# LPD-EPFL-ML/X-MAP

Measured on AMD Instinct MI355X. Metric: item_sim_pairs_per_s, higher is better.
Workload: dtype f64

## Files before the change

include/xmap_hip.h:

```cpp
#ifndef XMAP_HIP_H
#define XMAP_HIP_H
#include <stdint.h>

#ifdef __cplusplus
extern "C" {
#endif

#define XMAP_OK 0
#define XMAP_ERR_HIP -1
#define XMAP_ERR_ARG -2
#define XMAP_ERR_OVERFLOW -3
#define XMAP_ERR_CAPACITY -4

#define XMAP_COSINE 0
#define XMAP_ADJUST_COSINE 1
#define XMAP_COSINE_EXACT 2

#define XMAP_TOPC 10

typedef struct xmap_ratings {
    int64_t n_users;
    int32_t n_items;
    int64_t nnz;
    const int64_t *user_ptr;
    const int32_t *user_item;
    const float *user_rating;
    const int64_t *user_time;
    const int64_t *item_ptr;
    const int32_t *item_user;
    const float *item_rating;
    const int32_t *prefix_cls;
    const int32_t *suffix_cls;
    const uint32_t *contains_mask;
    const uint8_t *flags;
} xmap_ratings;

const char *xmap_last_error(void);
int xmap_version(void);

int xmap_trim(void);
int xmap_debug_arena(void *stream, int64_t *live, int64_t *reserved);
int xmap_debug_arena_call(void *stream, int64_t bytes, int fail);

int xmap_exclusive_scan_i64(void *stream, const int64_t *in, int64_t *out, int64_t n, int64_t *h_total);
int xmap_exclusive_scan_i32_to_i64(void *stream, const int32_t *in, int64_t *out, int64_t n, int64_t *h_total);


int xmap_build_csc(void *stream, int64_t n_users, int32_t n_items, int64_t nnz, const int64_t *user_ptr,
                   const int32_t *user_item, const float *user_rating, int32_t *cnt ,
                   int64_t *item_ptr , int32_t *item_user , float *item_rating );

int xmap_user_stats(void *stream, const xmap_ratings *R, double *u_avg, double *u_norm2);

int xmap_item_stats(void *stream, const xmap_ratings *R, const double *u_avg, double *info ,
                    double *norms ,
                    int32_t *ua_item , int32_t *ia_user ,
                    int32_t item_lo, int32_t item_hi );

#ifdef XMAP_CROSSCHECK
int xmap_sim_plan(void *stream, const xmap_ratings *R, int32_t slot_target, int32_t *Q, int64_t *W, int64_t *unit_ptr,
                  int64_t *h_n_units, int64_t *h_contrib);
int xmap_sim_units(void *stream, int32_t n_items, const int32_t *Q, const int64_t *unit_ptr,
                   int32_t *unit_item , int32_t *unit_q );

int xmap_sim_count(void *stream, const xmap_ratings *R, int method, int cap, const double *u_avg,
                   const double *info, const int32_t *ua_item, const int32_t *ia_user, const int32_t *Q,
                   const int32_t *unit_item, const int32_t *unit_q, int64_t unit_lo, int64_t unit_hi,
                   int32_t *unit_cnt , int64_t *d_counters , int64_t *h_counters );
int xmap_sim_fill(void *stream, const xmap_ratings *R, int method, int cap, const double *u_avg,
                  const double *info, const int32_t *ua_item, const int32_t *ia_user, const int32_t *Q,
                  const int32_t *unit_item, const int32_t *unit_q, int64_t unit_lo, int64_t unit_hi,
                  const int64_t *unit_off , int32_t *col, double *sim, int32_t *mutu, int32_t *nij);

int xmap_sim_row_ptr(void *stream, int32_t n_items, const int64_t *unit_ptr, const int64_t *unit_off ,
                     int64_t *row_ptr );
#endif

int xmap_sim2_layout(void *stream, const xmap_ratings *R, const double *info, int32_t ch_min, int32_t *hist ,
                     int64_t *pre , int32_t *ctl , int32_t *hid , int32_t *hlist ,
                     uint64_t *ub_key , void *ub ,
                     void *rc ,
                     uint64_t *Wp ,
                     int32_t dups , int32_t *h_ctl );
int xmap_sim2_plan(void *stream, const xmap_ratings *R, int32_t slot_target, const void *rc, const int64_t *pre,
                   const int32_t *hid, const int32_t *ctl, int32_t *Q, int32_t *C, uint8_t *small ,
                   uint64_t *Wp , int32_t *Qcat , int64_t *uq_ptr ,
                   int64_t *uc_ptr , int32_t dups, int64_t *h_counts );
int xmap_sim2_units(void *stream, int32_t n_items, const int64_t *item_ptr, const int32_t *Qcat, const int64_t *uq_ptr,
                    int32_t *uq_item, int32_t *uq_q , const int32_t *C, const int64_t *uc_ptr, int32_t *uc_item,
                    int32_t *uc_c);
int xmap_sim2_pairs(void *stream, const xmap_ratings *R, int method, int cap, const double *u_avg, const double *norms,
                    const void *rc, const void *ub, const int32_t *Q,
                    const uint8_t *small, const int32_t *uq_item, const int32_t *uq_q, const int64_t *cls_ptr ,
                    int64_t unit_lo, int64_t unit_hi, const int32_t *hid,
                    const int32_t *hlist, const int32_t *ctl, const int32_t *C, const int64_t *uc_ptr,
                    const int32_t *uc_item, const int32_t *uc_c, int32_t n_heavy_units, int32_t n_heavy, int phases,
                    double *hp_hi, double *hp_lo, int32_t *hp_cnt, int32_t *hp_mut, int64_t coo_cap, int32_t *coo_i,
                    int32_t *coo_j, double *coo_sim, int32_t *coo_mutu, int32_t *coo_nij,
                    double *coo_ls , int32_t *rowcnt,
                    int32_t *rowcnt_h , int64_t *d_shards ,
                    int64_t *d_counters ,
                    int32_t *mircnt );
int xmap_sim2_scatter(void *stream, int32_t n_items, int64_t n_coo, const int32_t *coo_i, const int32_t *coo_j,
                      const double *coo_sim, const int32_t *coo_mutu, const int32_t *coo_nij, const double *coo_ls ,
                      const int64_t *row_ptr, int32_t *fill , const int32_t *hid, const int32_t *hlist,
                      int32_t *col, double *sim, int32_t *mutu, int32_t *nij, double *ls );
int xmap_sim3_layout(void *stream, const xmap_ratings *R, int64_t *item_ptr ,
                     const double *rating64 , int32_t ch_min, int32_t phases, int32_t stats_lo, int32_t stats_hi,
                     int32_t *cnt ,
                     double *u_avg , double *u_norm , int32_t *hist ,
                     int64_t *pre , int32_t *ctl , int32_t *hid , int32_t *hlist ,
                     uint64_t *ub_key , void *ub , void *srec ,
                     void *bufA , void *bufB , void *rc ,
                     uint64_t *Wp , double *info , double *norms , int32_t *h_ctl );
int xmap_sim3_plan(void *stream, const xmap_ratings *R, int32_t slot_target, const int64_t *pre, const int32_t *hid,
                   const int32_t *ctl, int32_t *Q, int32_t *C, uint8_t *small, uint64_t *Wp, int32_t *Qcat ,
                   int64_t *uq_ptr , int64_t *uc_ptr , int32_t dups, int32_t *uq_item, int32_t *uq_q ,
                   int32_t *uc_item, int32_t *uc_c, int64_t cap_light, int64_t cap_heavy, int64_t *h_out );
int xmap_sim3_mircount(void *stream, int32_t n_items, int64_t coo_cap, const int32_t *coo_i, const int32_t *coo_j,
                       const int64_t *d_shards , int64_t n_pairs, int32_t skip_self, void *scratch, int32_t *mir );
int xmap_sim3_mirror(void *stream, int32_t n_items, int64_t coo_cap, const int32_t *coo_i, const int32_t *coo_j,
                     const double *coo_sim, const int32_t *coo_mutu, const int32_t *coo_nij,
                     const int64_t *d_shards ,
                     int64_t n_pairs, const int32_t *own , const int32_t *mir , int32_t *tot ,
                     int64_t *row_ptr , int64_t *mptr , int32_t *fill ,
                     void *bufA , void *bufB , int32_t *col,
                     double *sim, int32_t *mutu, int32_t *nij, const double *coo_aux , double *aux ,
                     int32_t row_lo, int32_t row_hi );

int xmap_sim2_pack_pairs(void *stream, int64_t n_coo, const int32_t *coo_i, const int32_t *coo_j, const double *coo_sim,
                         const int32_t *coo_mutu, const int32_t *coo_nij, int64_t *rec , int64_t *h_count);
int xmap_sim2_unpack_pairs(void *stream, int64_t n, const int64_t *rec , int32_t *coo_i, int32_t *coo_j, double *coo_sim,
                           int32_t *coo_mutu, int32_t *coo_nij);
int xmap_item_partials(void *stream, const xmap_ratings *R, const double *u_avg, double *partial );
int xmap_item_merge(void *stream, int32_t n_items, int32_t n_parts, const double *parts , double *info ,
                    double *norms );
int xmap_sim2_pack_partials(void *stream, int64_t n_coo, const int32_t *coo_i, const int32_t *coo_j, const double *coo_hi,
                            const double *coo_lo, const int32_t *coo_mutu, const int32_t *coo_nij, int64_t *rec ,
                            int64_t *h_count);
int xmap_sim2_sort_partials(void *stream, int64_t n, const int64_t *rec , int64_t *rec_sorted , int32_t n_items,
                            int32_t n_owners );
int xmap_sim2_merge_partials(void *stream, int method, int cap, int32_t n_items, int64_t n, const int64_t *rec_sorted,
                             const double *norms , int32_t *coo_i, int32_t *coo_j, double *coo_sim, int32_t *coo_mutu,
                             int32_t *coo_nij, int32_t *rowcnt , int64_t *h_counts );



typedef struct xmap_sim {
    int32_t n_items;
    const int64_t *row_ptr;
    const int32_t *col;
    const double *sim;
    const int32_t *mutu;
    const int32_t *nij;
    const double *info;
    const double *frac;
} xmap_sim;

int xmap_bridge_flags(void *stream, const xmap_sim *S, const int32_t *prefix_cls, uint8_t *bb);

int xmap_knn_classify(void *stream, const xmap_sim *S, int top_k, const uint8_t *bb, const int32_t *suffix_cls,
                      const uint32_t *contains_mask, uint8_t *cls, int32_t *kcnt ,
                      int32_t *kcol , double *kval ,
                      int32_t row_lo, int32_t row_hi );

int xmap_knn_thresholds(void *stream, int32_t n_items, int top_k, const int32_t *kcnt, const int32_t *kcol, const double *kval,
                        void *thr );
int xmap_reverse_count(void *stream, const xmap_sim *S, int mode, int top_k, const uint8_t *bb, const uint8_t *cls,
                       const int32_t *kcnt, const int32_t *kcol, const double *kval, const int32_t *suffix_cls,
                       const uint32_t *contains_mask, const uint8_t *flags, const int64_t *attach_ptr,
                       const void *thr ,
                       int32_t *long_rows ,
                       uint8_t *eflag ,
                       int32_t *rcnt , int32_t row_lo, int32_t row_hi );
int xmap_reverse_count_att_rnn(void *stream, const xmap_sim *S, int top_k, const uint8_t *bb, const uint8_t *cls,
                               const int32_t *kcnt, const int32_t *kcol, const double *kval, const int32_t *suffix_cls,
                               const uint32_t *contains_mask, const uint8_t *flags, const void *thr, int32_t *long_rows,
                               uint8_t *eflag, int32_t *rcnt_att , int32_t *rcnt_rnn , int32_t row_lo, int32_t row_hi);
int xmap_reverse_fill(void *stream, const xmap_sim *S, int mode, int top_k, const uint8_t *bb, const uint8_t *cls,
                      const int32_t *kcnt, const int32_t *kcol, const double *kval, const int32_t *suffix_cls,
                      const uint32_t *contains_mask, const uint8_t *flags, const int64_t *attach_ptr,
                      const void *thr ,
                      int32_t *long_rows ,
                      uint8_t *eflag , const int64_t *rptr ,
                      int32_t *ridx, double *rval , uint8_t *rflag, int32_t row_lo, int32_t row_hi);

int xmap_path_weights(void *stream, int32_t n_items, int top_k, const uint8_t *cls, const int32_t *kcnt,
                      const int32_t *kcol, const uint8_t *flags, const int64_t *att_ptr, const int32_t *att_idx,
                      const int64_t *src_ptr, const int32_t *src_idx, const uint8_t *src_flag, const int64_t *rnn_ptr,
                      const int32_t *rnn_idx, int64_t *tmp , int64_t *paths );

int xmap_extend_paths(void *stream, int32_t n_items, int top_k, const uint8_t *cls, const int32_t *kcnt,
                      const int32_t *kcol, const double *kval, const uint8_t *flags, const int64_t *att_ptr,
                      const int32_t *att_idx, const double *att_val, const int64_t *src_ptr, const int32_t *src_idx,
                      const double *src_val, const uint8_t *src_flag, const int64_t *rnn_ptr, const int32_t *rnn_idx,
                      const double *rnn_val, int32_t n_units, const int32_t *unit_start, const int32_t *unit_c,
                      const int32_t *unit_G, const int32_t *unit_row, int32_t *unit_nt, int32_t n_heavy,
                      const int32_t *heavy_unit0, int32_t n_slots, double *acc, int32_t *touched, double *hacc,
                      int32_t *htouched, int32_t *n_cand, int32_t *top_end, double *top_val, int64_t xs_cap,
                      int64_t *xs_off, int32_t *xs_end, double *xs_val, int64_t *d_counters ,
                      int64_t *h_counters );
// ... 158 lines not shown
```

x-map_amd/csrc/api.hip:

```cpp
#include <math.h>
#include <stdlib.h>
#include <vector>

#include "common.h"

namespace xmap {

struct Pool {
    std::vector<void *> ptrs;
    void release() {
        for (void *p : ptrs) (void)hipFree(p);
        ptrs.clear();
    }
};

}

using namespace xmap;

struct xmap_ctx {
    int device = 0;
    hipStream_t st = nullptr;
    Pool p_ratings, p_sim, p_ext, p_gen, p_rows;
    xmap_ratings R;
// ... 177 lines not shown
        const double r = fabs((double)rating[k]);
        if (!(r <= 1e300)) return false;
        if (r > M) M = r;
        while (e <= 26 && ldexp(r, e) != floor(ldexp(r, e))) e++;
        if (e > 26) return false;
    }
    if (M == 0.0) return true;
    const double Mi = ldexp(M, e);
    if (Mi > 134217728.0) return false;
    const uint64_t m2 = (uint64_t)Mi * (uint64_t)Mi;
    return (uint64_t)U <= (1ull << 53) / m2;
}

int xmap_ctx_upload_ratings(xmap_ctx *c, int64_t n_users, int32_t n_items, const int64_t *user_ptr, const int32_t *item,
                            const float *rating, const int64_t *time, const int32_t *prefix_cls, const int32_t *suffix_cls,
                            const uint32_t *contains_mask, const uint8_t *flags) {
    XM_ARG(c && user_ptr && prefix_cls && suffix_cls && contains_mask && flags && n_users >= 0 && n_items >= 0);
    XM_HIP(hipSetDevice(c->device));
    drop_tail(c);
    c->p_gen.release(); c->p_ext.release(); c->p_sim.release(); c->p_ratings.release();
    c->have_sim = c->have_ext = c->have_gen = false;
    const int64_t nnz = user_ptr[n_users];
    XM_ARG(nnz >= 0 && nnz < 2147483647ll && (nnz == 0 || (item && rating && time)));
    for (int64_t e = 0; e < nnz; e++) XM_ARG(item[e] >= 0 && item[e] < n_items);
    xmap_ratings &R = c->R;
    memset(&R, 0, sizeof(R));
    R.n_users = n_users; R.n_items = n_items; R.nnz = nnz;
    c->half_contrib = 0;
    for (int64_t u = 0; u < n_users; u++) { const int64_t d = user_ptr[u + 1] - user_ptr[u]; c->half_contrib += d * (d - 1) / 2; }
    int64_t *d_ptr, *d_time, *d_iptr;
    int32_t *d_item, *d_iuser, *d_pre, *d_suf;
    float *d_rating, *d_irating;
    uint32_t *d_mask;
    uint8_t *d_flags;
    XM_TRY(h2d(c->p_ratings, &d_ptr, user_ptr, (size_t)n_users + 1, c->st));
    XM_TRY(h2d(c->p_ratings, &d_item, item, (size_t)nnz, c->st));
    XM_TRY(h2d(c->p_ratings, &d_rating, rating, (size_t)nnz, c->st));
    XM_TRY(h2d(c->p_ratings, &d_time, time, (size_t)nnz, c->st));
    XM_TRY(h2d(c->p_ratings, &d_pre, prefix_cls, (size_t)n_items, c->st));
    XM_TRY(h2d(c->p_ratings, &d_suf, suffix_cls, (size_t)n_items, c->st));
    XM_TRY(h2d(c->p_ratings, &d_mask, contains_mask, (size_t)n_items, c->st));
    XM_TRY(h2d(c->p_ratings, &d_flags, flags, (size_t)n_items, c->st));
    XM_ALLOCZ(c->p_ratings, d_iptr, n_items + 1);
    XM_ALLOCZ(c->p_ratings, d_iuser, nnz);
    XM_ALLOCZ(c->p_ratings, d_irating, nnz);
    R.user_ptr = d_ptr; R.user_item = d_item; R.user_rating = d_rating; R.user_time = d_time;
    R.item_ptr = d_iptr; R.item_user = d_iuser; R.item_rating = d_irating;
    R.prefix_cls = d_pre; R.suffix_cls = d_suf; R.contains_mask = d_mask; R.flags = d_flags;
    c->plain_exact = plain_sums_exact(n_users, nnz, rating);
    XM_HIP(hipStreamSynchronize(c->st));
    c->have_ratings = true;
    return XMAP_OK;
}

int xmap_ctx_item_sim(xmap_ctx *c, int method, int cap, int64_t *n_kept, int64_t *n_evaluated) {
    XM_ARG(c && c->have_ratings && (method == XMAP_COSINE || method == XMAP_ADJUST_COSINE) && cap > 0);
    XM_HIP(hipSetDevice(c->device));
    drop_tail(c);
    c->p_gen.release(); c->p_ext.release(); c->p_sim.release();
    c->have_sim = c->have_ext = c->have_gen = false;
    xmap_ratings &R = c->R;
    const int I = R.n_items;
    const int64_t U = R.n_users, nnz = R.nnz;
    const int pair_method = (method == XMAP_COSINE && !c->plain_exact) ? XMAP_COSINE_EXACT : method;
    Pool tmp;
    struct Guard { Pool &p; ~Guard() { p.release(); } } guard{tmp};
#define T_ALLOC(ptr, n) XM_TRY(dalloc(tmp, &(ptr), (size_t)(n), c->st))
#define T_ALLOCZ(ptr, n) XM_TRY(dalloc(tmp, &(ptr), (size_t)(n), c->st, true))
    int32_t *cnt;
    T_ALLOC(cnt, I);
    double *norms;
    XM_ALLOC(c->p_sim, c->u_avg, U);
    XM_ALLOC(c->p_sim, c->u_norm, U);
    XM_ALLOCZ(c->p_sim, c->info, (size_t)I * 4);
    T_ALLOCZ(norms, (size_t)2 * I);
    int32_t *hist, *ctl, *hid, *hlist;
    int64_t *pre;
    uint64_t *ub_key, *ub, *rcrec, *Wp, *srec, *buf_a, *buf_b;
    const size_t n1 = (size_t)(nnz ? nnz : 1);
    T_ALLOC(hist, U + 2); T_ALLOC(pre, U + 3); T_ALLOC(ctl, 4); T_ALLOC(hid, I); T_ALLOCZ(hlist, 1024);
    T_ALLOC(ub_key, n1); T_ALLOC(ub, n1); T_ALLOC(rcrec, 2 * n1); T_ALLOC(Wp, I);
    T_ALLOC(srec, 2 * n1); T_ALLOC(buf_a, 2 * n1); T_ALLOC(buf_b, 2 * n1);
    const int ch_min = 2048;
    XM_TRY(xmap_sim3_layout(c->st, &R, (int64_t *)R.item_ptr, nullptr, ch_min, 1 | 2 | 4, 0, I, cnt, c->u_avg, c->u_norm, hist, pre, ctl,
                            hid, hlist, ub_key, ub, srec, buf_a, buf_b, rcrec, Wp, c->info, norms, nullptr));
    const int64_t half_contrib = c->half_contrib;
    int32_t *Q, *Cc, *Qcat, *uq_item = nullptr, *uq_q = nullptr, *uc_item = nullptr, *uc_c = nullptr;
    uint8_t *small;
    int64_t *uq_ptr, *uc_ptr;
    T_ALLOCZ(Q, I); T_ALLOCZ(Cc, I); T_ALLOCZ(small, I); T_ALLOC(Qcat, (size_t)5 * (I ? I : 1)); T_ALLOCZ(uq_ptr, (size_t)5 * I + 1);
    T_ALLOCZ(uc_ptr, I + 1);
    int slot_target = 768;
    double coo_slack = 1.0;
    int64_t hc[10];
    int64_t n_light = 0, n_hu = 0;
    int n_heavy = 0;
    auto plan = [&](int target) -> int {
        const int64_t cap_light = half_contrib / target + I + 1, cap_heavy = nnz / ch_min + 1025;
        T_ALLOC(uq_item, cap_light); T_ALLOC(uq_q, 4 * cap_light); T_ALLOC(uc_item, cap_heavy); T_ALLOC(uc_c, cap_heavy);
        XM_TRY(xmap_sim3_plan(c->st, &R, target, pre, hid, ctl, Q, Cc, small, Wp, Qcat, uq_ptr, uc_ptr, 0, uq_item, uq_q, uc_item, uc_c,
                              cap_light, cap_heavy, hc));
        n_light = hc[0]; n_hu = hc[1]; n_heavy = (int)hc[9];
        return XMAP_OK;
    };
    XM_TRY(plan(slot_target));
    int32_t *coo_i = nullptr, *coo_j = nullptr, *coo_mutu = nullptr, *coo_nij = nullptr, *own = nullptr, *mir = nullptr;
    double *coo_sim = nullptr;
    int64_t *d_shards = nullptr;
    int64_t cap_coo = 0, n = 0, n_unordered = 0;
    for (;;) {
        cap_coo = ((int64_t)((double)(half_contrib > 0 ? half_contrib : 1) * coo_slack) / 4096 + 1100) * 4096;
        double *hp_hi, *hp_lo;
        int32_t *hp_cnt, *hp_mut, *rowcnt_h;
        int64_t *d_cnt;
        T_ALLOC(coo_i, cap_coo); T_ALLOC(coo_j, cap_coo); T_ALLOC(coo_sim, cap_coo); T_ALLOC(coo_mutu, cap_coo); T_ALLOC(coo_nij, cap_coo);
        T_ALLOC(own, I); T_ALLOC(mir, I);
        const size_t hp = (size_t)(n_hu ? n_hu : 1) * 1024;
        T_ALLOC(hp_hi, hp); T_ALLOC(hp_lo, hp); T_ALLOC(hp_cnt, hp); T_ALLOC(hp_mut, hp);
        T_ALLOCZ(d_cnt, 6); T_ALLOC(d_shards, 2 * 4096); T_ALLOC(rowcnt_h, 64 * 1024);
        XM_TRY(xmap_sim2_pairs(c->st, &R, pair_method, cap, c->u_avg, norms, rcrec, ub, Q, small, uq_item, uq_q, hc + 2, 0, n_light, hid, hlist,
                               ctl, Cc, uc_ptr, uc_item, uc_c, (int32_t)n_hu, n_heavy, 8 | 1 | 2 | 4 | 16 | 64 | 128, hp_hi, hp_lo, hp_cnt,
                               hp_mut, cap_coo, coo_i, coo_j, coo_sim, coo_mutu, coo_nij, nullptr, own, rowcnt_h, d_shards, d_cnt, mir));
        int64_t h_cnt[6];
        XM_TRY(d2h(h_cnt, d_cnt, 6, c->st));
        XM_HIP(hipStreamSynchronize(c->st));
        if (h_cnt[2]) {
            if (slot_target <= 32) { set_error("pair-table overflow"); return XMAP_ERR_OVERFLOW; }
            slot_target /= 2;
            XM_TRY(plan(slot_target));
            continue;
        }
        if (h_cnt[3]) {
            if (coo_slack > 64) { set_error("half-COO overflow"); return XMAP_ERR_CAPACITY; }
            coo_slack *= 2;
            continue;
        }
        n = h_cnt[4]; n_unordered = h_cnt[5];
        break;
    }
    int64_t *row_ptr, *mptr;
    XM_ALLOCZ(c->p_sim, row_ptr, I + 1);
    T_ALLOCZ(mptr, I + 1);
    const int64_t kept = 2 * n;
    int32_t *col, *mutu, *nij, *fill, *tot;
    double *sim;
    uint64_t *mir_a, *mir_b;
    XM_ALLOC(c->p_sim, col, kept); XM_ALLOC(c->p_sim, sim, kept); XM_ALLOC(c->p_sim, mutu, kept); XM_ALLOC(c->p_sim, nij, kept);
    T_ALLOC(fill, I); T_ALLOC(tot, I); T_ALLOC(mir_a, (size_t)3 * (n ? n : 1)); T_ALLOC(mir_b, (size_t)3 * (n ? n : 1));
    XM_TRY(xmap_sim3_mircount(c->st, I, cap_coo, coo_i, coo_j, d_shards, n, 0, mir_a, mir));
    XM_TRY(xmap_sim3_mirror(c->st, I, cap_coo, coo_i, coo_j, coo_sim, coo_mutu, coo_nij, d_shards, n, own, mir, tot, row_ptr, mptr, fill,
                            mir_a, mir_b, col, sim, mutu, nij, nullptr, nullptr, 0, I));
    XM_HIP(hipStreamSynchronize(c->st));
    c->S.n_items = I; c->S.row_ptr = row_ptr; c->S.col = col; c->S.sim = sim; c->S.mutu = mutu; c->S.nij = nij; c->S.info = c->info;
    c->S.frac = nullptr;
    c->n_kept = kept; c->n_eval = 2 * n_unordered; c->n_contrib = 2 * half_contrib;
    c->have_sim = true;
    if (n_kept) *n_kept = kept;
    if (n_evaluated) *n_evaluated = c->n_eval;
    return XMAP_OK;
#undef T_ALLOC
#undef T_ALLOCZ
}

int xmap_ctx_sim_download(xmap_ctx *c, int64_t *row_ptr, int32_t *col, double *sim, int32_t *mutu, int32_t *nij, double *info,
                          double *user_avg) {
    XM_ARG(c && c->have_sim);
    XM_HIP(hipSetDevice(c->device));
    const int I = c->R.n_items;
    if (row_ptr) XM_TRY(d2h(row_ptr, c->S.row_ptr, (size_t)I + 1, c->st));
    if (col) XM_TRY(d2h(col, c->S.col, (size_t)c->n_kept, c->st));
    if (sim) XM_TRY(d2h(sim, c->S.sim, (size_t)c->n_kept, c->st));
    if (mutu) XM_TRY(d2h(mutu, c->S.mutu, (size_t)c->n_kept, c->st));
    if (nij) XM_TRY(d2h(nij, c->S.nij, (size_t)c->n_kept, c->st));
    if (info) XM_TRY(d2h(info, (const double *)c->info, (size_t)I * 4, c->st));
    if (user_avg) XM_TRY(d2h(user_avg, (const double *)c->u_avg, (size_t)c->R.n_users, c->st));
    XM_HIP(hipStreamSynchronize(c->st));
    return XMAP_OK;
}

int xmap_ctx_extend(xmap_ctx *c, int top_k, int64_t *n_out, int64_t *n_paths) {
    XM_ARG(c && c->have_sim && top_k >= 1);
    XM_HIP(hipSetDevice(c->device));
    drop_tail(c);
    c->p_gen.release(); c->p_ext.release();
    c->have_ext = c->have_gen = false;
    const int I = c->R.n_items, k = top_k;
    c->top_k = k;
    xmap_ext_tables &T = c->T;
    memset(&T, 0, sizeof(T));
    T.n_items = I; T.top_k = k; T.flags = c->R.flags;
    XM_ALLOCZ(c->p_ext, c->n_cand, I);
    XM_ALLOC(c->p_ext, c->top_end, (size_t)I * XMAP_TOPC);
    XM_ALLOCZ(c->p_ext, c->top_val, (size_t)I * XMAP_TOPC);
    c->n_out = c->n_paths = 0;
    if (I == 0) { c->have_ext = true; if (n_out) *n_out = 0; if (n_paths) *n_paths = 0; return XMAP_OK; }
    uint8_t *bb, *cls;
    int32_t *kcnt, *kcol;
    double *kval;
    XM_ALLOCZ(c->p_ext, bb, I); XM_ALLOC(c->p_ext, cls, I); XM_ALLOC(c->p_ext, kcnt, (size_t)I * 2);
    XM_ALLOC(c->p_ext, kcol, (size_t)I * 2 * k); XM_ALLOC(c->p_ext, kval, (size_t)I * 2 * k * 3);
    XM_TRY(xmap_bridge_flags(c->st, &c->S, c->R.prefix_cls, bb));
    XM_TRY(xmap_knn_classify(c->st, &c->S, k, bb, c->R.suffix_cls, c->R.contains_mask, cls, kcnt, kcol, kval, 0, I));
    T.cls = cls; T.kcnt = kcnt; T.kcol = kcol; T.kval = kval;
    XM_TRY(xmap_edge_ranges(c->st, &c->S, &c->fast_div));
    double *thr;
    int32_t *long_rows;
    XM_ALLOC(c->p_ext, thr, (size_t)I * 4);
    XM_ALLOC(c->p_ext, long_rows, I + 1);
    uint8_t *eflag;
    XM_ALLOC(c->p_ext, eflag, (size_t)(c->n_kept > 0 ? c->n_kept : 1));
    XM_TRY(xmap_knn_thresholds(c->st, I, k, kcnt, kcol, kval, thr));
    const uint8_t *dummy;
    int32_t *cnt_att, *cnt_rnn;
    XM_ALLOCZ(c->p_ext, cnt_att, I);
    XM_ALLOCZ(c->p_ext, cnt_rnn, I);
    XM_TRY(xmap_reverse_count_att_rnn(c->st, &c->S, k, bb, cls, kcnt, kcol, kval, c->R.suffix_cls, c->R.contains_mask, c->R.flags,
                                      thr, long_rows, eflag, cnt_att, cnt_rnn, 0, I));
    XM_TRY(reverse_list(c, 0, bb, nullptr, thr, long_rows, eflag, cnt_att, &T.att_ptr, &T.att_idx, &T.att_val, &dummy));
    XM_TRY(reverse_list(c, 2, bb, nullptr, thr, long_rows, eflag, cnt_rnn, &T.rnn_ptr, &T.rnn_idx, &T.rnn_val, &dummy));
    XM_TRY(reverse_list(c, 1, bb, T.att_ptr, thr, long_rows, eflag, nullptr, &T.src_ptr, &T.src_idx, &T.src_val, &T.src_flag));
    int64_t *wtmp, *P;
    XM_ALLOCZ(c->p_ext, wtmp, (size_t)4 * I); XM_ALLOCZ(c->p_ext, P, I);
    XM_TRY(xmap_path_weights(c->st, I, k, cls, kcnt, kcol, c->R.flags, T.att_ptr, T.att_idx, T.src_ptr, T.src_idx, T.src_flag, T.rnn_ptr,
                             T.rnn_idx, wtmp, P));
    int32_t *nb_list, *nb_id;
    int64_t n_nb = 0;
    XM_ALLOC(c->p_ext, nb_list, I); XM_ALLOC(c->p_ext, nb_id, I);
    XM_TRY(xmap_nb_index(c->st, I, cls, nb_list, nb_id, &n_nb));
    T.n_nb = (int32_t)n_nb; T.nb_list = nb_list; T.nb_id = nb_id;
    if (n_nb > 0) {
        int32_t *ng;
        int64_t *nrec, *dir_ptr, *rec_ptr, n_tiles = 0, n_records = 0;
// ... 107 lines not shown
    const int64_t U = c->R.n_users;
    int32_t *d_top, *d_choice, *d_map, *d_picks = nullptr;
    XM_ALLOCZ(c->p_gen, d_top, I); XM_ALLOCZ(c->p_gen, d_choice, I); XM_ALLOCZ(c->p_gen, d_map, I);
    if (picks) XM_TRY(h2d(c->p_gen, &d_picks, picks, (size_t)I, c->st));
    XM_TRY(xmap_select_map(c->st, I, private_flag ? 1 : 0, c->n_cand, c->top_end, d_picks, d_top, d_choice, d_map));
    if (choice) XM_TRY(d2h(choice, (const int32_t *)d_choice, (size_t)I, c->st));
    int32_t *cnt_t, *cnt_m;
    int64_t *off_t, *off_m, nt = 0, nm = 0;
    XM_ALLOCZ(c->p_gen, cnt_t, U); XM_ALLOCZ(c->p_gen, cnt_m, U); XM_ALLOCZ(c->p_gen, off_t, U + 1); XM_ALLOCZ(c->p_gen, off_m, U + 1);
    XM_TRY(xmap_alterego_count(c->st, &c->R, d_map, cnt_t, cnt_m, nullptr));
    XM_TRY(xmap_exclusive_scan_i32_to_i64(c->st, cnt_t, off_t, U, &nt));
    XM_TRY(xmap_exclusive_scan_i32_to_i64(c->st, cnt_m, off_m, U, &nm));
    const int64_t n = nt + nm;
    XM_ALLOC(c->p_gen, c->g_user, n); XM_ALLOC(c->p_gen, c->g_item, n); XM_ALLOC(c->p_gen, c->g_rating, n); XM_ALLOC(c->p_gen, c->g_time, n);
    XM_TRY(xmap_alterego_fill(c->st, &c->R, d_map, off_t, off_m, nt, c->g_user, c->g_item, c->g_rating, c->g_time));
    XM_HIP(hipStreamSynchronize(c->st));
    c->n_rows = n; c->n_target_rows = nt;
    c->g_off_t = off_t; c->g_off_m = off_m;
    c->have_gen = true;
    if (n_rows) *n_rows = n;
    if (n_target_rows) *n_target_rows = nt;
    return XMAP_OK;
}

int xmap_ctx_gen_download(xmap_ctx *c, int32_t *user, int32_t *item, double *rating, int64_t *time) {
    XM_ARG(c && c->have_gen);
    XM_HIP(hipSetDevice(c->device));
    const size_t n = (size_t)c->n_rows;
    if (user) XM_TRY(d2h(user, (const int32_t *)c->g_user, n, c->st));
    if (item) XM_TRY(d2h(item, (const int32_t *)c->g_item, n, c->st));
    if (rating) XM_TRY(d2h(rating, (const double *)c->g_rating, n, c->st));
    if (time) XM_TRY(d2h(time, (const int64_t *)c->g_time, n, c->st));
    XM_HIP(hipStreamSynchronize(c->st));
    return XMAP_OK;
}


int xmap_ctx_rec_sim(xmap_ctx *c, int cap, int64_t *n_pairs) {
    XM_ARG(c && c->have_gen && cap > 0);
    XM_HIP(hipSetDevice(c->device));
    drop_tail(c);
    const int I = c->R.n_items;
    const int64_t U = c->R.n_users, nnz = c->n_rows;
    XM_ARG(nnz < 2147483647ll);
    const size_t n1 = (size_t)(nnz ? nnz : 1), i1 = (size_t)(I ? I : 1);
    XM_ALLOCZ(c->p_rec, c->pf_ptr, U + 1);
    XM_ALLOC(c->p_rec, c->pf_item, n1); XM_ALLOC(c->p_rec, c->pf_rating, n1); XM_ALLOC(c->p_rec, c->pf_time, n1);
    XM_TRY(xmap_rec_profiles(c->st, U, nnz, c->n_target_rows, c->g_off_t, c->g_off_m, c->g_user, c->g_item, c->g_rating, c->g_time,
                             c->pf_ptr, c->pf_item, c->pf_rating, c->pf_time));
    XM_ALLOCZ(c->p_rec, c->rs_row_ptr, I + 1);
    XM_ALLOCZ(c->p_rec, c->rs_avg, i1); XM_ALLOCZ(c->p_rec, c->rs_norm, i1);
    c->rec_pairs = 0;
    if (I == 0 || nnz == 0) {
        XM_HIP(hipStreamSynchronize(c->st));
        c->have_rec = true;
        if (n_pairs) *n_pairs = 0;
        return XMAP_OK;
    }
    std::vector<int64_t> h_ptr((size_t)U + 1);
    XM_TRY(d2h(h_ptr.data(), (const int64_t *)c->pf_ptr, (size_t)U + 1, c->st));
    XM_HIP(hipStreamSynchronize(c->st));
    int64_t half_contrib = 0;
    for (int64_t u = 0; u < U; u++) { const int64_t d = h_ptr[u + 1] - h_ptr[u]; half_contrib += d * (d - 1) / 2; }
    Pool tmp;
    struct Guard { Pool &p; ~Guard() { p.release(); } } guard{tmp};
#define T_ALLOC(ptr, n) XM_TRY(dalloc(tmp, &(ptr), (size_t)(n), c->st))
#define T_ALLOCZ(ptr, n) XM_TRY(dalloc(tmp, &(ptr), (size_t)(n), c->st, true))
    xmap_ratings P = c->R;
    float *f_dummy, *f_irating;
    int64_t *item_ptr;
    int32_t *i_user;
    T_ALLOCZ(f_dummy, n1); T_ALLOCZ(f_irating, n1); T_ALLOCZ(item_ptr, I + 1); T_ALLOCZ(i_user, n1);
    P.nnz = nnz; P.user_ptr = c->pf_ptr; P.user_item = c->pf_item; P.user_rating = f_dummy; P.user_time = c->pf_time;
    P.item_ptr = item_ptr; P.item_user = i_user; P.item_rating = f_irating;
    int32_t *cnt, *hist, *ctl, *hid, *hlist;
    int64_t *pre;
    uint64_t *ub_key, *ub, *rcrec, *Wp, *srec, *buf_a, *buf_b;
    double *u_avg, *info, *norms;
    T_ALLOC(cnt, i1); T_ALLOCZ(u_avg, U ? U : 1); T_ALLOCZ(info, i1 * 4); T_ALLOCZ(norms, 2 * i1);
    T_ALLOC(hist, U + 2); T_ALLOC(pre, U + 3); T_ALLOC(ctl, 4); T_ALLOC(hid, i1); T_ALLOCZ(hlist, 1024);
    T_ALLOC(ub_key, n1); T_ALLOC(ub, 2 * n1); T_ALLOC(rcrec, 2 * n1); T_ALLOC(Wp, i1);
    T_ALLOC(srec, 3 * n1); T_ALLOC(buf_a, 3 * n1); T_ALLOC(buf_b, 3 * n1);
    const int ch_min = (int)((U + 2 > 64) ? U + 2 : 64);
    XM_TRY(xmap_sim3_layout(c->st, &P, item_ptr, c->pf_rating, ch_min, 1 | 2 | 4, 0, I, cnt, u_avg, nullptr, hist, pre, ctl, hid, hlist,
                            ub_key, ub, srec, buf_a, buf_b, rcrec, Wp, info, norms, nullptr));
    int32_t *Q, *Cc, *Qcat, *uq_item = nullptr, *uq_q = nullptr, *uc_item = nullptr, *uc_c = nullptr;
    uint8_t *small;
    int64_t *uq_ptr, *uc_ptr;
    T_ALLOCZ(Q, i1); T_ALLOCZ(Cc, i1); T_ALLOCZ(small, i1); T_ALLOC(Qcat, 5 * i1); T_ALLOCZ(uq_ptr, (size_t)5 * I + 1);
    T_ALLOCZ(uc_ptr, I + 1);
    int slot_target = 768;
    double coo_slack = 1.0;
    int64_t hc[10];
    int64_t n_light = 0;
    auto plan = [&](int target) -> int {
        const int64_t cap_light = half_contrib / target + I + 1, cap_heavy = nnz / ch_min + 1025;
        T_ALLOC(uq_item, cap_light); T_ALLOC(uq_q, 4 * cap_light); T_ALLOC(uc_item, cap_heavy); T_ALLOC(uc_c, cap_heavy);
        XM_TRY(xmap_sim3_plan(c->st, &P, target, pre, hid, ctl, Q, Cc, small, Wp, Qcat, uq_ptr, uc_ptr, 1, uq_item, uq_q, uc_item, uc_c,
                              cap_light, cap_heavy, hc));
        n_light = hc[0];
        return XMAP_OK;
    };
    XM_TRY(plan(slot_target));
    int32_t *coo_i = nullptr, *coo_j = nullptr, *coo_mutu = nullptr, *coo_nij = nullptr, *own = nullptr, *mir = nullptr;
    double *coo_sim = nullptr, *coo_ls = nullptr;
    int64_t *d_shards = nullptr;
    int64_t cap_coo = 0, n = 0;
    for (;;) {
        cap_coo = ((int64_t)((double)(half_contrib > 0 ? half_contrib : 1) * coo_slack) / 4096 + 1100) * 4096;
        double *hp_hi, *hp_lo;
        int32_t *hp_cnt, *hp_mut, *rowcnt_h;
        int64_t *d_cnt;
        T_ALLOC(coo_i, cap_coo); T_ALLOC(coo_j, cap_coo); T_ALLOC(coo_sim, cap_coo); T_ALLOC(coo_mutu, cap_coo); T_ALLOC(coo_nij, cap_coo);
        T_ALLOC(coo_ls, cap_coo); T_ALLOC(own, i1); T_ALLOC(mir, i1);
        T_ALLOC(hp_hi, 1024); T_ALLOC(hp_lo, 1024); T_ALLOC(hp_cnt, 1024); T_ALLOC(hp_mut, 1024);
        T_ALLOCZ(d_cnt, 6); T_ALLOC(d_shards, 2 * 4096); T_ALLOC(rowcnt_h, 64 * 1024);
        XM_TRY(xmap_sim2_pairs(c->st, &P, XMAP_ADJUST_COSINE, cap, u_avg, norms, rcrec, ub, Q, small, uq_item, uq_q, hc + 2, 0, n_light, hid,
                               hlist, ctl, Cc, uc_ptr, uc_item, uc_c, 0, 0, 8 | 2 | 16 | 64 | 128, hp_hi, hp_lo, hp_cnt, hp_mut, cap_coo,
                               coo_i, coo_j, coo_sim, coo_mutu, coo_nij, coo_ls, own, rowcnt_h, d_shards, d_cnt, mir));
        int64_t h_cnt[6];
        XM_TRY(d2h(h_cnt, d_cnt, 6, c->st));
        XM_HIP(hipStreamSynchronize(c->st));
        if (h_cnt[2]) {
            if (slot_target <= 32) { set_error("pair-table overflow"); return XMAP_ERR_OVERFLOW; }
            slot_target /= 2;
            XM_TRY(plan(slot_target));
            continue;
        }
        if (h_cnt[3]) {
            if (coo_slack > 64) { set_error("half-COO overflow"); return XMAP_ERR_CAPACITY; }
            coo_slack *= 2;
            continue;
        }
        n = h_cnt[4];
        break;
    }
    int64_t *mptr;
    T_ALLOCZ(mptr, I + 1);
    const size_t kept_max = (size_t)(n ? 2 * n : 1), nn = (size_t)(n ? n : 1);
    int32_t *mutu, *fill, *tot;
    uint64_t *mir_a, *mir_b;
    XM_ALLOC(c->p_rec, c->rs_col, kept_max); XM_ALLOC(c->p_rec, c->rs_sim, kept_max); XM_ALLOC(c->p_rec, c->rs_nij, kept_max);
    XM_ALLOC(c->p_rec, c->rs_ls, kept_max);
    T_ALLOC(mutu, kept_max); T_ALLOC(fill, i1); T_ALLOC(tot, i1); T_ALLOC(mir_a, 4 * nn); T_ALLOC(mir_b, 4 * nn);
    XM_TRY(xmap_sim3_mircount(c->st, I, cap_coo, coo_i, coo_j, d_shards, n, 1, mir_a, mir));
    XM_TRY(xmap_sim3_mirror(c->st, I, cap_coo, coo_i, coo_j, coo_sim, coo_mutu, coo_nij, d_shards, n, own, mir, tot, c->rs_row_ptr, mptr, fill,
                            mir_a, mir_b, c->rs_col, c->rs_sim, mutu, c->rs_nij, coo_ls, c->rs_ls, 0, I));
    XM_HIP(hipMemcpy2DAsync(c->rs_avg, sizeof(double), info, 4 * sizeof(double), sizeof(double), (size_t)I, hipMemcpyDeviceToDevice, c->st));
    XM_HIP(hipMemcpyAsync(c->rs_norm, norms + I, sizeof(double) * (size_t)I, hipMemcpyDeviceToDevice, c->st));
    int64_t kept = 0;
    XM_TRY(d2h(&kept, (const int64_t *)(c->rs_row_ptr + I), 1, c->st));
    XM_HIP(hipStreamSynchronize(c->st));
    c->rec_pairs = kept;
    c->have_rec = true;
    if (n_pairs) *n_pairs = kept;
    return XMAP_OK;
#undef T_ALLOC
#undef T_ALLOCZ
}

int xmap_ctx_rec_profiles_download(xmap_ctx *c, int64_t *prof_ptr, int32_t *prof_item, double *prof_rating, int64_t *prof_time) {
    XM_ARG(c && c->have_rec);
    XM_HIP(hipSetDevice(c->device));
    const size_t n = (size_t)c->n_rows;
    if (prof_ptr) XM_TRY(d2h(prof_ptr, (const int64_t *)c->pf_ptr, (size_t)c->R.n_users + 1, c->st));
    if (prof_item) XM_TRY(d2h(prof_item, (const int32_t *)c->pf_item, n, c->st));
    if (prof_rating) XM_TRY(d2h(prof_rating, (const double *)c->pf_rating, n, c->st));
    if (prof_time) XM_TRY(d2h(prof_time, (const int64_t *)c->pf_time, n, c->st));
    XM_HIP(hipStreamSynchronize(c->st));
    return XMAP_OK;
}

int xmap_ctx_rec_download(xmap_ctx *c, int64_t *row_ptr, int32_t *col, double *sim, double *ls, int32_t *nij, double *item_avg,
                          double *item_norm) {
    XM_ARG(c && c->have_rec);
    XM_HIP(hipSetDevice(c->device));
    const size_t I = (size_t)c->R.n_items, n = (size_t)c->rec_pairs;
    if (row_ptr) XM_TRY(d2h(row_ptr, (const int64_t *)c->rs_row_ptr, I + 1, c->st));
    if (col) XM_TRY(d2h(col, (const int32_t *)c->rs_col, n, c->st));
    if (sim) XM_TRY(d2h(sim, (const double *)c->rs_sim, n, c->st));
    if (ls) XM_TRY(d2h(ls, (const double *)c->rs_ls, n, c->st));
    if (nij) XM_TRY(d2h(nij, (const int32_t *)c->rs_nij, n, c->st));
    if (item_avg) XM_TRY(d2h(item_avg, (const double *)c->rs_avg, I, c->st));
    if (item_norm) XM_TRY(d2h(item_norm, (const double *)c->rs_norm, I, c->st));
    XM_HIP(hipStreamSynchronize(c->st));
    return XMAP_OK;
}

static int alloc_neighbors(xmap_ctx *c, int keep) {
    c->p_nb.release();
    c->have_nb = false;
    const size_t m = (size_t)(c->R.n_items ? c->R.n_items : 1) * keep;
    XM_ALLOCZ(c->p_nb, c->nb_cnt, c->R.n_items ? c->R.n_items : 1);
    XM_ALLOCZ(c->p_nb, c->nb_col, m); XM_ALLOCZ(c->p_nb, c->nb_sim, m); XM_ALLOCZ(c->p_nb, c->nb_ls, m);
    c->keep = keep;
    return XMAP_OK;
}

int xmap_ctx_rec_select(xmap_ctx *c, int keep) {
    XM_ARG(c && c->have_rec && keep >= 1 && keep <= 64);
    XM_HIP(hipSetDevice(c->device));
    XM_TRY(alloc_neighbors(c, keep));
    if (c->rec_pairs > 0)
        XM_TRY(xmap_rec_select(c->st, c->R.n_items, c->rs_row_ptr, c->rs_col, c->rs_sim, c->rs_ls, keep, c->nb_cnt, c->nb_col, c->nb_sim,
                               c->nb_ls));
    XM_HIP(hipStreamSynchronize(c->st));
    c->have_nb = true;
    return XMAP_OK;
}

int xmap_ctx_rec_set_neighbors(xmap_ctx *c, int keep, const int32_t *cnt, const int32_t *col, const double *sim) {
    XM_ARG(c && c->have_rec && keep >= 1 && keep <= 64 && cnt && col && sim);
    XM_HIP(hipSetDevice(c->device));
    const int I = c->R.n_items;
    for (int i = 0; i < I; i++) {
        XM_ARG(cnt[i] <= keep);
        for (int t = 0; t < cnt[i]; t++) XM_ARG(col[(size_t)i * keep + t] >= 0 && col[(size_t)i * keep + t] < I);
    }
    XM_TRY(alloc_neighbors(c, keep));
    const size_t m = (size_t)I * keep;
    if (I) {
        XM_HIP(hipMemcpyAsync(c->nb_cnt, cnt, sizeof(int32_t) * (size_t)I, hipMemcpyHostToDevice, c->st));
        XM_HIP(hipMemcpyAsync(c->nb_col, col, sizeof(int32_t) * m, hipMemcpyHostToDevice, c->st));
        XM_HIP(hipMemcpyAsync(c->nb_sim, sim, sizeof(double) * m, hipMemcpyHostToDevice, c->st));
    }
    XM_HIP(hipStreamSynchronize(c->st));
    c->have_nb = true;
    return XMAP_OK;
// ... 49 lines not shown
```

x-map_amd/csrc/common.h:

```cpp
#pragma once
#if defined(__HIP_DEVICE_COMPILE__) && !defined(__gfx950__)
#error "libxmap_hip is written for gfx950 (MI355X): build with --offload-arch=gfx950"
#endif
#include <hip/hip_runtime.h>
#include <stdint.h>
#include <stdio.h>
#include <string.h>

#include "../../include/xmap_hip.h"

namespace xmap {

void set_error(const char *fmt, ...);

#define XM_HIP(call)                                                                         \
    do {                                                                                     \
        hipError_t e_ = (call);                                                              \
        if (e_ != hipSuccess) {                                                              \
            xmap::set_error("%s:%d %s -> %s", __FILE__, __LINE__, #call, hipGetErrorString(e_)); \
            return XMAP_ERR_HIP;                                                             \
        }                                                                                    \
    } while (0)

#define XM_LAUNCH_CHECK() XM_HIP(hipGetLastError())

#define XM_ARG(cond)                                                        \
    do {                                                                    \
        if (!(cond)) {                                                      \
            xmap::set_error("%s:%d bad argument: %s", __FILE__, __LINE__, #cond); \
            return XMAP_ERR_ARG;                                            \
        }                                                                   \
    } while (0)

hipError_t xm_malloc_async(void **p, size_t bytes, hipStream_t st);
hipError_t xm_free_async(void *p, hipStream_t st);
struct XmScope {
    int dev; hipStream_t st; size_t live0; bool ok;
    explicit XmScope(hipStream_t st);
    ~XmScope();
    XmScope(const XmScope &) = delete;
    XmScope &operator=(const XmScope &) = delete;
};
#define XM_SCOPE(stream) xmap::XmScope xm_scope_((hipStream_t)(stream))
int radix_sort_pairs(hipStream_t st, unsigned long long *keys, int *vals, unsigned long long *keys_tmp, int *vals_tmp, long long n,
                     int bits);

constexpr int WAVE = 64;

__device__ __forceinline__ int lane_id() { return threadIdx.x & 63; }

__device__ __forceinline__ int rl32(int v, int l) { return __builtin_amdgcn_readlane(v, l); }
__device__ __forceinline__ float rlf(float v, int l) { return __int_as_float(rl32(__float_as_int(v), l)); }
__device__ __forceinline__ long long rl64(long long v, int l) {
    int lo = rl32((int)(v & 0xffffffffll), l), hi = rl32((int)(v >> 32), l);
    return ((long long)hi << 32) | (unsigned int)lo;
}
__device__ __forceinline__ double rld(double v, int l) {
    return __longlong_as_double(rl64(__double_as_longlong(v), l));
}
__device__ __forceinline__ int uniform(int v) { return __builtin_amdgcn_readfirstlane(v); }

__device__ __forceinline__ unsigned long long lanemask_lt() {
    return (1ull << lane_id()) - 1ull;
}

__device__ __forceinline__ double wave_sum(double v) {
#pragma unroll
    for (int m = 32; m >= 1; m >>= 1) v += __shfl_xor(v, m, 64);
    return v;
}
__device__ __forceinline__ long long wave_sum_ll(long long v) {
#pragma unroll
    for (int m = 32; m >= 1; m >>= 1) v += __shfl_xor(v, m, 64);
    return v;
}

__device__ __forceinline__ void dd_add(double &hi, double &lo, double x) {
    double s = hi + x;
    double bb = s - hi;
    double e = (hi - (s - bb)) + (x - bb);
    e += lo;
    double h2 = s + e;
    lo = e - (h2 - s);
    hi = h2;
}

template <int G>
__device__ __forceinline__ void dd_reduce(double &hi, double &lo) {
#pragma unroll
    for (int m = G / 2; m >= 1; m >>= 1) {
        double oh = __shfl_down(hi, m, G), ol = __shfl_down(lo, m, G);
        dd_add(hi, lo, oh);
        dd_add(hi, lo, ol);
    }
}

__device__ __forceinline__ uint32_t mix32(uint32_t h) {
    h ^= h >> 16; h *= 0x85EBCA6Bu; h ^= h >> 13; h *= 0xC2B2AE35u; h ^= h >> 16;
    return h;
}

}
```

x-map_amd/csrc/stage_a2.hip:

```cpp
#include <type_traits>

#include "common.h"
#include "item_stats.h"
#include "tilesort.h"

namespace xmap {

constexpr int T_LOG_SLOTS = 10;
constexpr int T_SLOTS = 1 << T_LOG_SLOTS;
constexpr int HMAX = 1024;
constexpr uint32_t T_EMPTY = 0xFFFFFFFFu;
constexpr int SMALL_BOUND = 96;
constexpr int MID_BOUND = 384;

constexpr int N_CLASSES = 5;
constexpr int WIDE_MIN = 2048;
__host__ __device__ __forceinline__ int class_rank(int cls) {
    return cls == 4 ? 0 : (cls == 0 ? 1 : (cls == 2 ? 2 : (cls == 3 ? 3 : 4)));
}

__device__ __forceinline__ unsigned long long wkey(int n, int item) {
    return ((unsigned long long)(unsigned)n << 32) | (unsigned)item;
}

// ... 923 lines not shown
    }
    base = ((unsigned long long)(unsigned)rl32((int)(base >> 32), 0) << 32) | (unsigned)rl32((int)(base & 0xffffffffull), 0);
    if (!keep) return;
    const long long p = (long long)base + __popcll(km & lanemask_lt());
    coo_i[p] = i; coo_j[p] = j; coo_sim[p] = simv; coo_mutu[p] = mm; coo_nij[p] = nn;
    atomicAdd(&rowcnt[i], 1);
    atomicAdd(&rowcnt[j], 1);
}


constexpr int CNT_SLOTS = 4096;
constexpr int CNT_CHUNK = 8192;
__device__ __forceinline__ int cnt_slot(int it) { return (int)(mix32((uint32_t)it) & (CNT_SLOTS - 1)); }

__global__ __launch_bounds__(256) void k_count3(long long nnz, const int *uitem, int *cnt) {
    __shared__ int tag[CNT_SLOTS], loc[CNT_SLOTS];
    for (int t = threadIdx.x; t < CNT_SLOTS; t += 256) { tag[t] = -1; loc[t] = 0; }
    __syncthreads();
    const long long e0 = (long long)blockIdx.x * CNT_CHUNK;
    for (int q = threadIdx.x; q < CNT_CHUNK; q += 256) {
        const long long e = e0 + q;
        if (e >= nnz) break;
        const int it = uitem[e];
        const int sl = cnt_slot(it);
        const int old = atomicCAS(&tag[sl], -1, it);
        if (old == -1 || old == it) atomicAdd(&loc[sl], 1); else atomicAdd(&cnt[it], 1);
    }
    __syncthreads();
    for (int t = threadIdx.x; t < CNT_SLOTS; t += 256)
        if (loc[t]) atomicAdd(&cnt[tag[t]], loc[t]);
}

constexpr int CB_MAX = 1024;
constexpr int CB_CHUNK = 8192;
constexpr int CB_WIN = 8192;
constexpr int CB_SPB = 4;
constexpr int CB_T = 1024;

__global__ __launch_bounds__(CB_MAX) void k_cb_scan(const unsigned *bcnt, long long *bptr, unsigned *bcur) {
    __shared__ long long ws[CB_MAX / 64];
    const int t = threadIdx.x, lane = t & 63, w = t >> 6;
    const long long c = bcnt[t];
    long long inc = c;
#pragma unroll
    for (int d = 1; d < 64; d <<= 1) { const long long o = __shfl_up(inc, d, 64); if (lane >= d) inc += o; }
    if (lane == 63) ws[w] = inc;
    __syncthreads();
    long long base = 0;
    for (int x = 0; x < w; x++) base += ws[x];
    bptr[t] = base + inc - c;
    if (t == CB_MAX - 1) bptr[CB_MAX] = base + inc;
    bcur[t] = 0u;
}

__global__ __launch_bounds__(CB_T) void k_cb_count(long long nnz, const int *part, int sh, const long long *bptr, int n_items, int *cnt) {
    __shared__ unsigned win[CB_WIN];
    __shared__ int s_b;
    if (nnz < 0) nnz = bptr[CB_MAX];
    const long long p0 = (long long)blockIdx.x * (CB_CHUNK * CB_SPB);
    if (p0 >= nnz) return;
    if (threadIdx.x == 0) {
        int lo = 0, hi = CB_MAX;
        while (hi - lo > 1) { const int mid = (lo + hi) >> 1; if (bptr[mid] <= p0) lo = mid; else hi = mid; }
        s_b = lo;
    }
    for (int t = threadIdx.x; t < CB_WIN; t += CB_T) win[t] = 0u;
    __syncthreads();
    const int item0 = s_b << sh;
#pragma unroll 4
    for (int q = threadIdx.x; q < CB_CHUNK * CB_SPB; q += CB_T) {
        const long long p = p0 + q;
        if (p >= nnz) break;
        const int it = part[p];
        const unsigned d = (unsigned)(it - item0);
        if (d < (unsigned)CB_WIN) atomicAdd(&win[d], 1u); else atomicAdd(&cnt[it], 1);
    }
    __syncthreads();
    for (int t = threadIdx.x; t < CB_WIN; t += CB_T)
        if (win[t] && item0 + t < n_items) atomicAdd(&cnt[item0 + t], (int)win[t]);
}

template <bool SELF>
__global__ __launch_bounds__(CB_T) void k_cbs_hist(long long range_cap, int n_ranges, const unsigned long long *cur, const int *coo_i,
                                                   const int *coo_j, int sh, unsigned *bcnt) {
    __shared__ unsigned h[CB_MAX];
    for (int t = threadIdx.x; t < CB_MAX; t += CB_T) h[t] = 0u;
    __syncthreads();
    const long long cpr = (range_cap + CB_CHUNK - 1) / CB_CHUNK;
#pragma unroll
    for (int sg = 0; sg < CB_SPB; sg++) {
        const long long g = (long long)blockIdx.x * CB_SPB + sg;
        const long long c = g / n_ranges;
        const int r = (int)(g - c * n_ranges);
        if (c >= cpr) break;
        const long long n = (cur && (long long)cur[r] < range_cap) ? (long long)cur[r] : range_cap;
        const long long b = (long long)r * range_cap;
#pragma unroll
        for (int q = 0; q < CB_CHUNK / CB_T; q++) {
            const long long e = c * CB_CHUNK + q * CB_T + threadIdx.x;
            if (e < n) {
                const int j = coo_j[b + e];
                if (!SELF || j != coo_i[b + e]) atomicAdd(&h[j >> sh], 1u);
            }
        }
    }
    __syncthreads();
    for (int t = threadIdx.x; t < CB_MAX; t += CB_T)
        if (h[t]) atomicAdd(&bcnt[t], h[t]);
}

template <bool SELF>
__global__ __launch_bounds__(CB_T) void k_cbs_scatter(long long range_cap, int n_ranges, const unsigned long long *cur, const int *coo_i,
                                                      const int *coo_j, int sh, const long long *bptr, unsigned *bcur, int *out) {
    static_assert(CB_T == CB_MAX, "one thread per bucket in the scan");
    __shared__ unsigned h[CB_MAX], off[CB_MAX + 1], wsum[CB_T / 64];
    __shared__ long long base[CB_MAX];
    __shared__ int stage[CB_CHUNK * CB_SPB];
    const int tid = threadIdx.x;
    h[tid] = 0u;
    __syncthreads();
    constexpr int EPT = CB_CHUNK / CB_T;
    const long long cpr = (range_cap + CB_CHUNK - 1) / CB_CHUNK;
    int it[CB_SPB][EPT];
    unsigned rk[CB_SPB][EPT];
#pragma unroll
    for (int sg = 0; sg < CB_SPB; sg++) {
        const long long g = (long long)blockIdx.x * CB_SPB + sg;
        const long long c = g / n_ranges;
        const int r = (int)(g - c * n_ranges);
        const long long n = (c < cpr) ? ((cur && (long long)cur[r] < range_cap) ? (long long)cur[r] : range_cap) : 0;
        const long long b = (long long)r * range_cap;
#pragma unroll
        for (int q = 0; q < EPT; q++) {
            const long long e = c * CB_CHUNK + q * CB_T + tid;
            it[sg][q] = -1;
            if (e < n) {
                const int j = coo_j[b + e];
                if (!SELF || j != coo_i[b + e]) it[sg][q] = j;
            }
        }
    }
#pragma unroll
    for (int sg = 0; sg < CB_SPB; sg++)
#pragma unroll
        for (int q = 0; q < EPT; q++) rk[sg][q] = it[sg][q] >= 0 ? atomicAdd(&h[it[sg][q] >> sh], 1u) : 0u;
    __syncthreads();
    {
        const unsigned c = h[tid];
        const int lane = tid & 63, w = tid >> 6;
        unsigned inc = c;
#pragma unroll
        for (int d = 1; d < 64; d <<= 1) { const unsigned o = __shfl_up(inc, d, 64); if (lane >= d) inc += o; }
        if (lane == 63) wsum[w] = inc;
        __syncthreads();
        unsigned bs = 0;
        for (int x = 0; x < w; x++) bs += wsum[x];
        off[tid] = bs + inc - c;
        if (tid == CB_T - 1) off[CB_MAX] = bs + inc;
        if (c) base[tid] = bptr[tid] + (long long)atomicAdd(&bcur[tid], c);
    }
    __syncthreads();
#pragma unroll
    for (int sg = 0; sg < CB_SPB; sg++)
#pragma unroll
        for (int q = 0; q < EPT; q++)
            if (it[sg][q] >= 0) stage[off[it[sg][q] >> sh] + rk[sg][q]] = it[sg][q];
    __syncthreads();
    const int total = (int)off[CB_MAX];
    for (int x = tid; x < total; x += CB_T) {
        const int v = stage[x];
        const int bk = v >> sh;
        out[base[bk] + (x - (int)off[bk])] = v;
    }
}


template <bool WIDE>
__device__ __forceinline__ void sort_entry3(const int *uitem, const float *ur32, const double *ur64, const int *cnt,
                                            long long e, unsigned long long &key, int &px, long long &py) {
    const int it = uitem[e];
    key = wkey(cnt[it], it);
    px = it;
    py = WIDE ? __double_as_longlong(ur64[e]) : (long long)(unsigned)__float_as_int(ur32[e]);
}

template <bool WIDE>
__device__ __forceinline__ void bitonic_desc3(int width, int pos, unsigned long long &key, int &px, long long &py) {
#pragma unroll
    for (int k2 = 2; k2 <= 64; k2 <<= 1) {
        if (k2 <= width)
#pragma unroll
        for (int j = k2 >> 1; j > 0; j >>= 1) {
            const unsigned long long ok = __shfl_xor(key, j, 64);
            const int ox = __shfl_xor(px, j, 64);
            long long oy;
            if (WIDE) oy = __shfl_xor(py, j, 64); else oy = (long long)(unsigned)__shfl_xor((int)py, j, 64);
            const bool desc = (pos & k2) == 0;
            const bool lower = (pos & j) == 0;
            const bool take_other = (lower == desc) ? (ok > key) : (ok < key);
            if (take_other) { key = ok; px = ox; py = oy; }
        }
    }
}

template <bool WIDE>
__device__ __forceinline__ void emit_entry3(long long a, int d, int rank, long long u, int px, long long py, void *ub,
                                            unsigned long long *srec) {
    const long long e = a + rank;
    const unsigned pos_ge = (unsigned)(d >= 2 ? rank : 0) | ((unsigned)px & 0x80000000u);
    const unsigned long long w0 = (unsigned long long)((unsigned)px & 0x7fffffffu) | ((unsigned long long)pos_ge << 32);
    if (WIDE) {
        UbWide v; v.item_ge = px; v.pad = 0; v.rating = __longlong_as_double(py);
        ((UbWide *)ub)[e] = v;
        srec[e * 3 + 0] = w0; srec[e * 3 + 1] = (unsigned long long)py; srec[e * 3 + 2] = (unsigned long long)(unsigned)u;
    } else {
        ((int2 *)ub)[e] = make_int2(px, (int)py);
        ulonglong2 w; w.x = w0; w.y = (unsigned long long)(unsigned)py | ((unsigned long long)(unsigned)u << 32);
        *(ulonglong2 *)(srec + e * 2) = w;
    }
}

// ... 471 lines not shown
    G.K = K; G.M = M; G.ch = ch;
    G.ts_log = 11;
    for (;;) {
        const long long TS = 1ll << G.ts_log;
        long long kw = M / (4 * (long long)(K > 0 ? K : 1));
        const long long kw_min = TS / (ts::NK_MAX - 2) + 1;
        if (kw < kw_min) kw = kw_min;
        if (kw < 4) kw = 4;
        const long long tiles = ((M + (long long)K * kw) >> G.ts_log) + 1;
        if (tiles <= (long long)ts::NA_MAX * ts::NB || G.ts_log >= 30) {
            G.KW = (int)kw;
            G.NA = (int)((tiles + ts::NB - 1) / ts::NB);
            if (G.NA < 1) G.NA = 1;
            if (G.NA > ts::NA_MAX) G.NA = ts::NA_MAX;
            G.T = G.NA * ts::NB;
            return;
        }
        G.ts_log++;
    }
}

int ts_prepare(hipStream_t st, ts::Geo &G, const long long *ptr) {
    G.ptr = ptr;
    G.clist_cap = G.M / G.ch + G.NA + 1;
    G.slist_cap = G.M / ts::SL + (G.M >> G.ts_log) + 2;
    XM_HIP(xm_malloc_async((void **)&G.tk, sizeof(unsigned) * (size_t)(G.K > 0 ? G.K : 1), st));
    XM_HIP(xm_malloc_async((void **)&G.tile_key0, sizeof(int) * ((size_t)G.T + 1), st));
    XM_HIP(xm_malloc_async((void **)&G.tile_pos0, sizeof(long long) * ((size_t)G.T + 1), st));
    XM_HIP(xm_malloc_async((void **)&G.tile_large, sizeof(int) * (size_t)G.T, st));
    unsigned long long *z = nullptr;
    const size_t nz = (size_t)G.NA + 2 * (size_t)G.T + 1;
    XM_HIP(xm_malloc_async((void **)&z, sizeof(unsigned long long) * nz, st));
    G.curA = z; G.curB = z + G.NA; G.counters = (unsigned *)(z + G.NA + 2 * (size_t)G.T);
    XM_HIP(xm_malloc_async((void **)&G.clist, sizeof(int2) * (size_t)G.clist_cap, st));
    XM_HIP(xm_malloc_async((void **)&G.slist, sizeof(int2) * (size_t)G.slist_cap, st));
    XM_HIP(hipMemsetAsync(z, 0, sizeof(unsigned long long) * nz, st));
    XM_HIP(hipMemsetAsync(G.tile_large, 0xff, sizeof(int) * (size_t)G.T, st));
    ts::k_ts_plan<<<dim3((unsigned)((G.K + 255) / 256)), dim3(256), 0, st>>>(G);
    XM_LAUNCH_CHECK();
    ts::k_ts_chunks<<<dim3((unsigned)((G.NA + 255) / 256)), dim3(256), 0, st>>>(G);
    XM_LAUNCH_CHECK();
    return XMAP_OK;
}
}

namespace {
template <bool AUX, bool SHARE>
int mirror_levels(hipStream_t st, const ts::Geo &G, int64_t coo_cap, const int32_t *coo_i, const int32_t *coo_j, const double *coo_sim,
                  const int32_t *coo_mutu, const int32_t *coo_nij, const double *coo_aux, const longlong2 *chunks, const unsigned *n_chunks,
                  long long chunk_cap, int64_t n_pairs, const int32_t *own, const int64_t *row_ptr, int32_t *fill, void *bufA, void *bufB,
                  int32_t *col, double *sim, int32_t *mutu, int32_t *nij, double *aux, int row_lo, int row_hi) {
    constexpr int RW = AUX ? 4 : 3;
    CooLoaderT<AUX, SHARE> LA{coo_i, coo_j, coo_sim, coo_mutu, coo_nij, coo_aux, chunks, n_chunks, (const long long *)row_ptr, fill,
                              col, sim, mutu, nij, aux, row_lo, row_hi};
    ts::RecLoader<RW> LB{(const unsigned long long *)bufA};
    ts::k_ts_bin<RW, false, CooLoaderT<AUX, SHARE>><<<dim3((unsigned)chunk_cap), dim3(ts::BT), 0, st>>>(G, LA, coo_cap, (unsigned long long *)bufA);
    XM_LAUNCH_CHECK();
    ts::k_ts_bin<RW, true, ts::RecLoader<RW>><<<dim3((unsigned)G.clist_cap), dim3(ts::BT), 0, st>>>(G, LB, n_pairs, (unsigned long long *)bufB);
    XM_LAUNCH_CHECK();
    k_mir_tiles<AUX><<<dim3((unsigned)G.T), dim3(ts::CT), 0, st>>>(G, (const unsigned long long *)bufB, (const long long *)row_ptr, own, col,
                                                                   sim, mutu, nij, aux);
    XM_LAUNCH_CHECK();
    k_mir_large<AUX><<<dim3((unsigned)G.slist_cap), dim3(ts::LT), 0, st>>>(G, (const unsigned long long *)bufB, (const long long *)row_ptr, own,
                                                                            col, sim, mutu, nij, aux);
    XM_LAUNCH_CHECK();
    return XMAP_OK;
}
}

namespace {
int mirror_counts(hipStream_t st, int n_items, long long range_cap, int n_ranges, const unsigned long long *cur, const int *coo_i,
                  const int *coo_j, bool skip_self, int *part, int *counts) {
    if (n_items <= 0 || range_cap <= 0 || n_ranges <= 0) return XMAP_OK;
    int sh = 0;
    while (((long long)(n_items - 1) >> sh) >= CB_MAX) sh++;
    unsigned *bcnt = nullptr, *bcur = nullptr;
    long long *bptr = nullptr;
    XM_HIP(xm_malloc_async((void **)&bcnt, sizeof(unsigned) * CB_MAX, st));
    XM_HIP(xm_malloc_async((void **)&bcur, sizeof(unsigned) * CB_MAX, st));
    XM_HIP(xm_malloc_async((void **)&bptr, sizeof(long long) * (CB_MAX + 1), st));
    XM_HIP(hipMemsetAsync(bcnt, 0, sizeof(unsigned) * CB_MAX, st));
    const long long segs = (long long)n_ranges * ((range_cap + CB_CHUNK - 1) / CB_CHUNK);
    const dim3 g((unsigned)((segs + CB_SPB - 1) / CB_SPB));
    if (skip_self) k_cbs_hist<true><<<g, dim3(CB_T), 0, st>>>(range_cap, n_ranges, cur, coo_i, coo_j, sh, bcnt);
    else k_cbs_hist<false><<<g, dim3(CB_T), 0, st>>>(range_cap, n_ranges, cur, coo_i, coo_j, sh, bcnt);
    XM_LAUNCH_CHECK();
    k_cb_scan<<<dim3(1), dim3(CB_MAX), 0, st>>>(bcnt, bptr, bcur);
    XM_LAUNCH_CHECK();
    if (skip_self) k_cbs_scatter<true><<<g, dim3(CB_T), 0, st>>>(range_cap, n_ranges, cur, coo_i, coo_j, sh, bptr, bcur, part);
    else k_cbs_scatter<false><<<g, dim3(CB_T), 0, st>>>(range_cap, n_ranges, cur, coo_i, coo_j, sh, bptr, bcur, part);
    XM_LAUNCH_CHECK();
    const long long cap = range_cap * n_ranges;
    k_cb_count<<<dim3((unsigned)((cap + (long long)CB_CHUNK * CB_SPB - 1) / ((long long)CB_CHUNK * CB_SPB))), dim3(CB_T), 0, st>>>(
        -1, part, sh, bptr, n_items, counts);
    XM_LAUNCH_CHECK();
    return XMAP_OK;
}
}

extern "C" {

int xmap_sim2_layout(void *stream, const xmap_ratings *R, const double *info, int32_t ch_min, int32_t *hist ,
                     int64_t *pre , int32_t *ctl , int32_t *hid, int32_t *hlist ,
                     uint64_t *ub_key , void *ub , void *rc ,
                     uint64_t *Wp , int32_t dups, int32_t *h_ctl ) {
    XM_ARG(R && info && hist && pre && ctl && hid && hlist && ub_key && ub && rc && Wp && ch_min >= 64);
    XM_ARG(R->nnz < 0x7fffffffLL && R->n_users < 0x7ffffff0LL);
    hipStream_t st = (hipStream_t)stream;
    const int I = R->n_items;
    const int HB = (int)R->n_users + 2;
    XM_HIP(hipMemsetAsync(hist, 0, sizeof(int32_t) * (size_t)HB, st));
    XM_HIP(hipMemsetAsync(ctl, 0x7f, sizeof(int32_t), st));
    XM_HIP(hipMemsetAsync(ctl + 1, 0, 3 * sizeof(int32_t), st));
    if (I > 0) {
        k_hist<<<dim3((unsigned)((I + 256 * HIST_PER - 1) / (256 * HIST_PER))), dim3(256), 0, st>>>(
            I, (const long long *)R->item_ptr, HB, hist);
        XM_LAUNCH_CHECK();
    }
    int rcode = xmap_exclusive_scan_i32_to_i64(stream, hist, pre, HB, nullptr);
    if (rcode) return rcode;
    if (HB - 1 > ch_min) {
        k_threshold<<<dim3((unsigned)((HB + 255) / 256)), dim3(256), 0, st>>>(I, HB, (const long long *)pre, ch_min, ctl);
        XM_LAUNCH_CHECK();
    }
    if (I > 0) {
        k_mark_heavy<<<dim3((unsigned)((I + 255) / 256)), dim3(256), 0, st>>>(I, (const long long *)R->item_ptr, ctl, hid,
                                                                                hlist, ctl + 1);
        XM_LAUNCH_CHECK();
    }
    if (R->n_users > 0) {
        k_sort_profiles<<<dim3((unsigned)((R->n_users + 15) / 16)), dim3(256), 0, st>>>(
            R->n_users, (const long long *)R->user_ptr, R->user_item, R->user_rating, (const long long *)R->item_ptr, info,
            (unsigned long long *)ub_key, (int2 *)ub);
        XM_LAUNCH_CHECK();
    }
    XM_HIP(hipMemsetAsync(Wp, 0, sizeof(uint64_t) * (size_t)(I > 0 ? I : 1), st));
    if (R->nnz > 0) {
        if (dups) XM_HIP(hipMemsetAsync(ub_key, 0, sizeof(int32_t) * (size_t)R->nnz, st));
        k_rater_records<<<dim3((unsigned)((R->nnz + 255) / 256)), dim3(256), 0, st>>>(
            I, R->nnz, (const long long *)R->item_ptr, R->item_user, (const long long *)R->user_ptr, (const int2 *)ub,
            (RaterRec *)rc, dups ? (int *)ub_key : nullptr, (unsigned long long *)Wp);
        XM_LAUNCH_CHECK();
    }
    if (h_ctl) {
        XM_HIP(hipMemcpyAsync(h_ctl, ctl, 2 * sizeof(int32_t), hipMemcpyDeviceToHost, st));
        XM_HIP(hipStreamSynchronize(st));
        if (h_ctl[1] > HMAX) {
            set_error("heavy set larger than %d", HMAX);
            return XMAP_ERR_OVERFLOW;
        }
    }
    return XMAP_OK;
}

int xmap_sim2_plan(void *stream, const xmap_ratings *R, int32_t slot_target, const void *rc, const int64_t *pre,
                   const int32_t *hid, const int32_t *ctl, int32_t *Q, int32_t *C, uint8_t *small, uint64_t *Wp ,
                   int32_t *Qcat , int64_t *uq_ptr , int64_t *uc_ptr, int32_t dups,
                   int64_t *h_counts ) {
    XM_ARG(R && rc && Wp && pre && hid && ctl && Q && C && small && Qcat && uq_ptr && uc_ptr && h_counts);
    XM_ARG(slot_target > 0 && slot_target <= T_SLOTS);
    hipStream_t st = (hipStream_t)stream;
    const int I = R->n_items;
    XM_HIP(hipMemsetAsync(Qcat, 0, sizeof(int32_t) * (size_t)N_CLASSES * (size_t)(I > 0 ? I : 1), st));
    if (I > 0) {
        k_plan2<<<dim3((unsigned)((I + 255) / 256)), dim3(256), 0, st>>>(
            I, (const long long *)R->item_ptr, (const RaterRec *)rc, (const long long *)pre, (int)R->n_users + 2, hid, ctl,
            slot_target, dups, Q, C, small, (unsigned long long *)Wp, Qcat);
        XM_LAUNCH_CHECK();
    }
    int rcode = xmap_exclusive_scan_i32_to_i64(stream, Qcat, uq_ptr, (int64_t)N_CLASSES * I, &h_counts[0]);
    if (rcode) return rcode;
    rcode = xmap_exclusive_scan_i32_to_i64(stream, C, uc_ptr, I, &h_counts[1]);
    if (rcode) return rcode;
    if (I > 0)
        XM_HIP(hipMemcpy2DAsync(&h_counts[2], sizeof(int64_t), uq_ptr, sizeof(int64_t) * (size_t)I, sizeof(int64_t),
                                N_CLASSES, hipMemcpyDeviceToHost, st));
    else
        for (int c = 0; c < N_CLASSES; c++) h_counts[2 + c] = 0;
    XM_HIP(hipStreamSynchronize(st));
    h_counts[2 + N_CLASSES] = h_counts[0];
    return XMAP_OK;
}

int xmap_sim2_units(void *stream, int32_t n_items, const int64_t *item_ptr, const int32_t *Qcat, const int64_t *uq_ptr,
                    int32_t *uq_item, int32_t *uq_q, const int32_t *C, const int64_t *uc_ptr, int32_t *uc_item, int32_t *uc_c) {
    XM_ARG(item_ptr && Qcat && uq_ptr && uq_item && uq_q && C && uc_ptr && uc_item && uc_c);
    if (n_items == 0) return XMAP_OK;
    k_fill_units2<<<dim3((unsigned)(((long long)N_CLASSES * n_items + 255) / 256)), dim3(256), 0, (hipStream_t)stream>>>(
        n_items, (const long long *)item_ptr, Qcat, (const long long *)uq_ptr, uq_item, uq_q, C, (const long long *)uc_ptr, uc_item, uc_c, 0x7fffffffffffffffLL,
        0x7fffffffffffffffLL);
    XM_LAUNCH_CHECK();
    return XMAP_OK;
}

int xmap_sim3_plan(void *stream, const xmap_ratings *R, int32_t slot_target, const int64_t *pre, const int32_t *hid,
                   const int32_t *ctl, int32_t *Q, int32_t *C, uint8_t *small, uint64_t *Wp, int32_t *Qcat, int64_t *uq_ptr,
                   int64_t *uc_ptr, int32_t dups, int32_t *uq_item, int32_t *uq_q, int32_t *uc_item, int32_t *uc_c,
                   int64_t cap_light, int64_t cap_heavy, int64_t *h_out) {
    XM_SCOPE(stream);
    XM_ARG(R && Wp && pre && hid && ctl && Q && C && small && Qcat && uq_ptr && uc_ptr && h_out);
    XM_ARG(uq_item && uq_q && uc_item && uc_c && cap_light >= 0 && cap_heavy >= 0);
    XM_ARG(slot_target > 0 && slot_target <= T_SLOTS);
    hipStream_t st = (hipStream_t)stream;
    const int I = R->n_items;
    for (int c = 0; c < 10; c++) h_out[c] = 0;
    XM_HIP(hipMemsetAsync(Qcat, 0, sizeof(int32_t) * (size_t)N_CLASSES * (size_t)(I > 0 ? I : 1), st));
    if (I > 0) {
        k_plan2<<<dim3((unsigned)((I + 255) / 256)), dim3(256), 0, st>>>(
            I, (const long long *)R->item_ptr, nullptr, (const long long *)pre, (int)R->n_users + 2, hid, ctl, slot_target, dups, Q, C,
            small, (unsigned long long *)Wp, Qcat);
        XM_LAUNCH_CHECK();
    }
    int rcode = xmap_exclusive_scan_i32_to_i64(stream, Qcat, uq_ptr, (int64_t)N_CLASSES * I, nullptr);
    if (rcode) return rcode;
    rcode = xmap_exclusive_scan_i32_to_i64(stream, C, uc_ptr, I, nullptr);
    if (rcode) return rcode;
    if (I > 0) {
        k_fill_units2<<<dim3((unsigned)(((long long)N_CLASSES * I + 255) / 256)), dim3(256), 0, st>>>(
            I, (const long long *)R->item_ptr, Qcat, (const long long *)uq_ptr, uq_item, uq_q, C, (const long long *)uc_ptr, uc_item, uc_c,
            cap_light, cap_heavy);
        XM_LAUNCH_CHECK();
        XM_HIP(hipMemcpy2DAsync(&h_out[2], sizeof(int64_t), uq_ptr, sizeof(int64_t) * (size_t)I, sizeof(int64_t), N_CLASSES + 1,
                                hipMemcpyDeviceToHost, st));
        XM_HIP(hipMemcpyAsync(&h_out[1], uc_ptr + I, sizeof(int64_t), hipMemcpyDeviceToHost, st));
    }
    int32_t h_ctl[2] = {0, 0};
    XM_HIP(hipMemcpyAsync(h_ctl, ctl, 2 * sizeof(int32_t), hipMemcpyDeviceToHost, st));
    XM_HIP(hipStreamSynchronize(st));
    h_out[0] = h_out[2 + N_CLASSES];
    h_out[8] = h_ctl[0]; h_out[9] = h_ctl[1];
    if (h_ctl[1] > HMAX) {
        set_error("heavy set larger than %d", HMAX);
        return XMAP_ERR_OVERFLOW;
    }
    if (h_out[0] > cap_light || h_out[1] > cap_heavy) {
        set_error("unit arrays too small: %lld light / %lld heavy units, room for %lld / %lld", (long long)h_out[0], (long long)h_out[1],
                  (long long)cap_light, (long long)cap_heavy);
        return XMAP_ERR_CAPACITY;
    }
    return XMAP_OK;
}

int xmap_sim2_pairs(void *stream, const xmap_ratings *R, int method, int cap, const double *u_avg, const double *norms,
                    const void *rc, const void *ub, const int32_t *Q,
                    const uint8_t *small, const int32_t *uq_item, const int32_t *uq_q, const int64_t *cls_ptr ,
                    int64_t unit_lo, int64_t unit_hi, const int32_t *hid,
                    const int32_t *hlist, const int32_t *ctl, const int32_t *C, const int64_t *uc_ptr,
                    const int32_t *uc_item, const int32_t *uc_c, int32_t n_heavy_units, int32_t n_heavy, int phases,
                    double *hp_hi, double *hp_lo, int32_t *hp_cnt, int32_t *hp_mut, int64_t coo_cap, int32_t *coo_i,
                    int32_t *coo_j, double *coo_sim, int32_t *coo_mutu, int32_t *coo_nij, double *coo_ls ,
                    int32_t *rowcnt, int32_t *rowcnt_h , int64_t *d_shards ,
                    int64_t *d_counters , int32_t *mircnt ) {
    XM_SCOPE(stream);
    XM_ARG(R && u_avg && norms && rc && ub);
    XM_ARG(Q && small && uq_item && uq_q && cls_ptr && hid && hlist && ctl && C && uc_ptr && uc_item && uc_c);
    XM_ARG(coo_i && coo_j && coo_sim && coo_mutu && coo_nij && rowcnt && rowcnt_h && d_shards && d_counters);
    XM_ARG(coo_cap >= COO_SHARDS);
    XM_ARG(method == XMAP_COSINE || method == XMAP_ADJUST_COSINE || method == XMAP_COSINE_EXACT);
    XM_ARG(n_heavy_units == 0 || !(phases & 5) || (hp_hi && hp_lo && hp_cnt && hp_mut));
    hipStream_t st = (hipStream_t)stream;
    const bool exact_cos = method == XMAP_COSINE_EXACT;
    const double *nrm = norms + (method == XMAP_ADJUST_COSINE ? (size_t)R->n_items : 0);
    if (exact_cos) {
        double *zero_avg = nullptr;
        const size_t ub = sizeof(double) * (size_t)(R->n_users > 0 ? R->n_users : 1);
        XM_HIP(xm_malloc_async((void **)&zero_avg, ub, st));
        XM_HIP(hipMemsetAsync(zero_avg, 0, ub, st));
        u_avg = zero_avg;
        method = XMAP_ADJUST_COSINE;
    }
    const bool raw = (phases & 32) != 0;
    XM_ARG(!coo_ls || ((raw || method == XMAP_ADJUST_COSINE) && n_heavy_units == 0));
    XM_ARG(!raw || (coo_ls && n_heavy_units == 0 && n_heavy == 0));
    if (phases & 8) {
        XM_HIP(hipMemsetAsync(d_counters, 0, 4 * sizeof(int64_t), st));
        XM_HIP(hipMemsetAsync(d_shards, 0, 2 * COO_SHARDS * sizeof(int64_t), st));
        if (!(phases & 128)) XM_HIP(hipMemsetAsync(coo_i, 0xff, sizeof(int32_t) * (size_t)coo_cap, st));
        XM_HIP(hipMemsetAsync(rowcnt, 0, sizeof(int32_t) * (size_t)(R->n_items > 0 ? R->n_items : 1), st));
        if (mircnt) XM_HIP(hipMemsetAsync(mircnt, 0, sizeof(int32_t) * (size_t)(R->n_items > 0 ? R->n_items : 1), st));
    }
    TriArgs A;
    memset(&A, 0, sizeof(A));
    A.iptr = (const long long *)R->item_ptr; A.rc = (const RaterRec *)rc; A.ub = (const int2 *)ub;
    A.u_avg = u_avg; A.nrm = nrm; A.cap = cap;
    A.Q = Q; A.small = small; A.uq_item = uq_item; A.uq_q = uq_q; A.unit_lo = unit_lo; A.unit_hi = unit_hi;
    A.hid = hid; A.hlist = hlist; A.CH = ctl; A.uc_item = uc_item; A.uc_c = uc_c;
    A.uc_ptr = (const long long *)uc_ptr; A.C = C;
    A.hp_hi = hp_hi; A.hp_lo = hp_lo; A.hp_cnt = hp_cnt; A.hp_mut = hp_mut;
    A.shard_cap = coo_cap / COO_SHARDS; A.shard_cur = (unsigned long long *)d_shards;
    A.shard_occ = (unsigned long long *)d_shards + COO_SHARDS; A.coo_i = coo_i; A.coo_j = coo_j; A.coo_sim = coo_sim; A.coo_mutu = coo_mutu; A.coo_nij = coo_nij;
    A.coo_aux = coo_ls;
    A.raw = raw ? 1 : 0;
    A.heavy_mod = (phases >> 16) & 0xff; A.heavy_rem = (phases >> 8) & 0xff;
    if (A.heavy_mod < 1) A.heavy_mod = 1;
    A.rowcnt = rowcnt; A.mircnt = mircnt; A.rowcnt_h = rowcnt_h; A.counters = (unsigned long long *)d_counters;
    const bool heavy_aside = (phases & 7) == 7 && n_heavy_units > 0 && unit_hi > unit_lo;
    hipStream_t hs = st;
    SideStreams *side = nullptr;
    if (((phases & 2) && unit_hi > unit_lo) || heavy_aside) {
        side = side_streams();
        if (!side) return XMAP_ERR_HIP;
        XM_HIP(hipEventRecord(side->fork, st));
    }
    if (heavy_aside) {
        hs = side->s[N_CLASSES];
        XM_HIP(hipStreamWaitEvent(hs, side->fork, 0));
    }
    if ((phases & 1) && n_heavy_units > 0) {
        if (method == XMAP_COSINE) k_pair_heavy<XMAP_COSINE><<<dim3((unsigned)n_heavy_units), dim3(64 * HEAVY_WAVES), 0, hs>>>(A);
        else k_pair_heavy<XMAP_ADJUST_COSINE><<<dim3((unsigned)n_heavy_units), dim3(64 * HEAVY_WAVES), 0, hs>>>(A);
        XM_LAUNCH_CHECK();
    }
    if (heavy_aside && n_heavy > 0) {
        if (method == XMAP_COSINE) k_heavy_merge<XMAP_COSINE><<<dim3((unsigned)n_heavy), dim3(256), 0, hs>>>(A, n_heavy);
        else k_heavy_merge<XMAP_ADJUST_COSINE><<<dim3((unsigned)n_heavy), dim3(256), 0, hs>>>(A, n_heavy);
        XM_LAUNCH_CHECK();
    }
    if (heavy_aside) {
        XM_HIP(hipEventRecord(side->done[N_CLASSES], hs));
        XM_HIP(hipStreamWaitEvent(st, side->done[N_CLASSES], 0));
    }
    if ((phases & 2) && unit_hi > unit_lo) {
        for (int c = 0; c < N_CLASSES; c++) {
// ... 262 lines not shown
            XM_LAUNCH_CHECK();
        }
    }
    }
    if ((phases & 2) && stats_hi > stats_lo) {
        BigList B;
        B.chunk_cap = nnz / STAT_CHK + nnz / STAT_BIG + 2;
        B.item_cap = nnz / STAT_BIG + 2;
        XM_HIP(xm_malloc_async((void **)&B.counters, 2 * sizeof(unsigned), st));
        XM_HIP(xm_malloc_async((void **)&B.chunks, sizeof(int2) * (size_t)B.chunk_cap, st));
        XM_HIP(xm_malloc_async((void **)&B.items, sizeof(int4) * (size_t)B.item_cap, st));
        XM_HIP(xm_malloc_async((void **)&B.part, sizeof(double) * ITEM_PART * (size_t)B.chunk_cap, st));
        XM_HIP(hipMemsetAsync(B.counters, 0, 2 * sizeof(unsigned), st));
        const dim3 grid((unsigned)((stats_hi - stats_lo + 15) / 16)), gridC((unsigned)((B.chunk_cap + 3) / 4)), gridI((unsigned)((B.item_cap + 63) / 64));
        if (wide) {
            const RcWideSrc src{(const RaterRecWide *)rc};
            k_item_stats3<RcWideSrc><<<grid, dim3(256), 0, st>>>(I, stats_lo, stats_hi, (const long long *)item_ptr, src, info, norms, B);
            XM_LAUNCH_CHECK();
            k_item_chunks<RcWideSrc><<<gridC, dim3(256), 0, st>>>((const long long *)item_ptr, src, B);
            XM_LAUNCH_CHECK();
            k_item_big<<<gridI, dim3(64), 0, st>>>(I, B, info, norms);
            XM_LAUNCH_CHECK();
        } else {
            const RcSrc src{(RaterRec *)rc, u_avg};
            k_item_stats3<RcSrc><<<grid, dim3(256), 0, st>>>(I, stats_lo, stats_hi, (const long long *)item_ptr, src, info, norms, B);
            XM_LAUNCH_CHECK();
            k_item_chunks<RcSrc><<<gridC, dim3(256), 0, st>>>((const long long *)item_ptr, src, B);
            XM_LAUNCH_CHECK();
            k_item_big<<<gridI, dim3(64), 0, st>>>(I, B, info, norms);
            XM_LAUNCH_CHECK();
            k_item_big_flags<RcSrc><<<gridC, dim3(256), 0, st>>>((const long long *)item_ptr, src, B, info);
            XM_LAUNCH_CHECK();
        }
    }
    if (!wide && nnz > 0 && I > 0) {
        if (phases & 8) {
            k_rc_flags<<<dim3((unsigned)((nnz + 255) / 256)), dim3(256), 0, st>>>(nnz, (RaterRec *)rc, (const int2 *)ub, info);
            XM_LAUNCH_CHECK();
        }
        if (phases & 4) {
            k_ub_flags<<<dim3((unsigned)((nnz + 255) / 256)), dim3(256), 0, st>>>(nnz, (int2 *)ub, info);
            XM_LAUNCH_CHECK();
        }
    }
    if (h_ctl) {
        XM_HIP(hipMemcpyAsync(h_ctl, ctl, 2 * sizeof(int32_t), hipMemcpyDeviceToHost, st));
        XM_HIP(hipStreamSynchronize(st));
        if (h_ctl[1] > HMAX) {
            set_error("heavy set larger than %d", HMAX);
            return XMAP_ERR_OVERFLOW;
        }
    }
    return XMAP_OK;
}

int xmap_sim3_mircount(void *stream, int32_t n_items, int64_t coo_cap, const int32_t *coo_i, const int32_t *coo_j,
                       const int64_t *d_shards, int64_t n_pairs, int32_t skip_self, void *scratch, int32_t *mir) {
    XM_SCOPE(stream);
    XM_ARG(coo_i && coo_j && scratch && mir && n_items >= 0 && coo_cap >= 0 && n_pairs >= 0);
    XM_ARG(d_shards ? (coo_cap >= COO_SHARDS) : (n_pairs <= coo_cap));
    hipStream_t st = (hipStream_t)stream;
    if (n_items == 0) return XMAP_OK;
    XM_HIP(hipMemsetAsync(mir, 0, sizeof(int32_t) * (size_t)n_items, st));
    if (n_pairs == 0 || coo_cap == 0) return XMAP_OK;
    if (d_shards)
        return mirror_counts(st, n_items, coo_cap / COO_SHARDS, COO_SHARDS, (const unsigned long long *)d_shards, coo_i, coo_j,
                             skip_self != 0, (int *)scratch, mir);
    return mirror_counts(st, n_items, n_pairs, 1, nullptr, coo_i, coo_j, skip_self != 0, (int *)scratch, mir);
}

int xmap_sim3_mirror(void *stream, int32_t n_items, int64_t coo_cap, const int32_t *coo_i, const int32_t *coo_j,
                     const double *coo_sim, const int32_t *coo_mutu, const int32_t *coo_nij, const int64_t *d_shards, int64_t n_pairs,
                     const int32_t *own, const int32_t *mir, int32_t *tot, int64_t *row_ptr, int64_t *mptr, int32_t *fill,
                     void *bufA, void *bufB, int32_t *col, double *sim, int32_t *mutu, int32_t *nij, const double *coo_aux, double *aux,
                     int32_t row_lo, int32_t row_hi) {
    XM_SCOPE(stream);
    XM_ARG(row_lo >= 0 && row_lo <= row_hi && row_hi <= n_items);
    XM_ARG(coo_i && coo_j && coo_sim && coo_mutu && coo_nij && own && mir && tot && row_ptr && mptr && fill && bufA && bufB);
    XM_ARG(col && sim && mutu && nij && n_items >= 0 && coo_cap >= 0 && n_pairs >= 0 && n_pairs < 0x7fffffffLL);
    XM_ARG(d_shards ? (coo_cap >= COO_SHARDS) : (n_pairs <= coo_cap));
    XM_ARG((coo_aux != nullptr) == (aux != nullptr));
    hipStream_t st = (hipStream_t)stream;
    const int I = n_items;
    if (I > 0) {
        k_row_totals<<<dim3((unsigned)((I + 255) / 256)), dim3(256), 0, st>>>(I, own, mir, tot);
        XM_LAUNCH_CHECK();
    }
    int rcode = xmap_exclusive_scan_i32_to_i64(stream, tot, row_ptr, I, nullptr);
    if (rcode) return rcode;
    rcode = xmap_exclusive_scan_i32_to_i64(stream, mir, mptr, I, nullptr);
    if (rcode) return rcode;
    if (n_pairs == 0 || I == 0 || coo_cap == 0) return XMAP_OK;
    XM_HIP(hipMemsetAsync(fill, 0, sizeof(int32_t) * (size_t)I, st));
    ts::Geo G;
    ts_geometry(I, n_pairs, coo_aux ? ts::Chunk<4>::CH : ts::Chunk<3>::CH, G);
    rcode = ts_prepare(st, G, (const long long *)mptr);
    if (rcode) return rcode;
    static_assert(ts::Chunk<3>::CH <= ts::Chunk<4>::CH && ts::Chunk<4>::CH % ts::Chunk<3>::CH == 0, "chunk lists by the narrow record width");
    const int n_shards = d_shards ? COO_SHARDS : 1;
    const long long shard_cap = d_shards ? coo_cap / COO_SHARDS : coo_cap;
    const long long chunk_cap = n_pairs / ts::Chunk<3>::CH + n_shards + 1;
    longlong2 *chunks = nullptr;
    unsigned *n_chunks = nullptr;
    XM_HIP(xm_malloc_async((void **)&chunks, sizeof(longlong2) * (size_t)chunk_cap, st));
    XM_HIP(xm_malloc_async((void **)&n_chunks, sizeof(unsigned), st));
    XM_HIP(hipMemsetAsync(n_chunks, 0, sizeof(unsigned), st));
    k_coo_chunks<<<dim3((unsigned)((n_shards + 255) / 256)), dim3(256), 0, st>>>(n_shards, shard_cap, (const unsigned long long *)d_shards,
                                                                                 n_pairs, chunks, n_chunks, chunk_cap);
    XM_LAUNCH_CHECK();
    const bool share = row_lo > 0 || row_hi < I;
#define XM_MIRROR(AUX_, SHARE_, CA_, A_) mirror_levels<AUX_, SHARE_>(st, G, coo_cap, coo_i, coo_j, coo_sim, coo_mutu, coo_nij, CA_, chunks, n_chunks, \
        chunk_cap, n_pairs, own, row_ptr, fill, bufA, bufB, col, sim, mutu, nij, A_, row_lo, row_hi)
    if (coo_aux) return share ? XM_MIRROR(true, true, coo_aux, aux) : XM_MIRROR(true, false, coo_aux, aux);
    return share ? XM_MIRROR(false, true, nullptr, nullptr) : XM_MIRROR(false, false, nullptr, nullptr);
#undef XM_MIRROR
}
}
```

x-map_amd/csrc/util.hip:

```cpp
#include <stdarg.h>
#include <stdlib.h>
#include <vector>

#include "common.h"

namespace xmap {
static thread_local char g_err[512] = "";
void set_error(const char *fmt, ...) {
    va_list ap;
    va_start(ap, fmt);
    vsnprintf(g_err, sizeof(g_err), fmt, ap);
    va_end(ap);
}

namespace {
struct Chunk { char *base; size_t size, used; };
struct Arena { int dev; hipStream_t st; std::vector<Chunk> chunks; size_t live; };
thread_local std::vector<Arena> g_arenas;
constexpr size_t ARENA_KEEP = (size_t)256 << 20;
Arena *arena_find(int dev, hipStream_t st) {
    for (Arena &a : g_arenas) if (a.dev == dev && a.st == st) return &a;
    return nullptr;
}
Arena *arena_of(hipStream_t st) {
    int dev = 0;
    if (hipGetDevice(&dev) != hipSuccess) return nullptr;
    if (Arena *a = arena_find(dev, st)) return a;
    g_arenas.push_back(Arena{dev, st, {}, 0});
    return &g_arenas.back();
}
void arena_reset(Arena *a) {
    size_t total = 0;
    for (Chunk &c : a->chunks) { c.used = 0; total += c.size; }
    if (total <= ARENA_KEEP) return;
    if (hipStreamSynchronize(a->st) != hipSuccess) return;
    std::vector<Chunk> keep;
    size_t kept = 0;
    std::vector<Chunk> all = a->chunks;
    for (size_t i = 0; i < all.size(); i++)
        for (size_t j = i + 1; j < all.size(); j++)
            if (all[j].size < all[i].size) { Chunk t = all[i]; all[i] = all[j]; all[j] = t; }
    for (Chunk &c : all) {
        if (kept + c.size <= ARENA_KEEP) { keep.push_back(c); kept += c.size; }
        else (void)hipFree(c.base);
    }
    a->chunks.swap(keep);
}
}

XmScope::XmScope(hipStream_t s) : dev(0), st(s), live0(0), ok(false) {
    if (hipGetDevice(&dev) != hipSuccess) return;
    ok = true;
    if (Arena *a = arena_find(dev, st)) live0 = a->live;
}
XmScope::~XmScope() {
    if (!ok) return;
    Arena *a = arena_find(dev, st);
    if (!a || a->live <= live0) return;
    a->live = live0;
    if (a->live == 0) arena_reset(a);
}

hipError_t xm_malloc_async(void **p, size_t bytes, hipStream_t st) {
    Arena *a = arena_of(st);
    if (!a) return hipErrorInvalidDevice;
    bytes = (bytes + 255) & ~(size_t)255;
    if (bytes == 0) bytes = 256;
    for (Chunk &c : a->chunks)
        if (c.size - c.used >= bytes) { *p = c.base + c.used; c.used += bytes; a->live++; return hipSuccess; }
    Chunk c;
    c.size = bytes > ((size_t)32 << 20) ? bytes : ((size_t)32 << 20);
    c.used = bytes;
    hipError_t e = hipMalloc((void **)&c.base, c.size);
    if (e != hipSuccess) return e;
    a->chunks.push_back(c);
    *p = c.base;
    a->live++;
    return hipSuccess;
}
hipError_t xm_free_async(void *p, hipStream_t st) {
    (void)p;
    Arena *a = arena_of(st);
    if (!a || a->live == 0) return hipErrorInvalidValue;
    if (--a->live == 0) arena_reset(a);
    return hipSuccess;
}

constexpr int SCAN_THREADS = 256;
constexpr int SCAN_ITEMS = 8;
constexpr int SCAN_TILE = SCAN_THREADS * SCAN_ITEMS;

__device__ __forceinline__ long long block_exclusive_scan(long long v, long long *total, long long *smem) {
    int lane = threadIdx.x & 63, w = threadIdx.x >> 6;
    long long inc = v;
#pragma unroll
    for (int d = 1; d < 64; d <<= 1) {
        long long o = __shfl_up(inc, d, 64);
        if (lane >= d) inc += o;
    }
    if (lane == 63) smem[w] = inc;
    __syncthreads();
    long long base = 0, tot = 0;
    for (int k = 0; k < SCAN_THREADS / 64; k++) {
        long long s = smem[k];
        if (k < w) base += s;
        tot += s;
    }
    __syncthreads();
    *total = tot;
    return base + inc - v;
}

template <typename TIn>
__global__ __launch_bounds__(SCAN_THREADS) void k_tile_sums(const TIn *in, long long n, long long *tile_sum) {
    __shared__ long long smem[4];
    long long base = (long long)blockIdx.x * SCAN_TILE + (long long)threadIdx.x * SCAN_ITEMS;
    long long s = 0;
#pragma unroll
    for (int k = 0; k < SCAN_ITEMS; k++)
        if (base + k < n) s += (long long)in[base + k];
    long long tot;
    block_exclusive_scan(s, &tot, smem);
    if (threadIdx.x == 0) tile_sum[blockIdx.x] = tot;
}

__global__ __launch_bounds__(SCAN_THREADS) void k_scan_tile_sums(long long *tile_sum, long long n_tiles, long long *grand) {
    __shared__ long long smem[4];
    long long carry = 0;
    for (long long b = 0; b < n_tiles; b += SCAN_THREADS) {
        long long i = b + threadIdx.x;
        long long v = i < n_tiles ? tile_sum[i] : 0;
        long long tot;
        long long ex = block_exclusive_scan(v, &tot, smem);
        if (i < n_tiles) tile_sum[i] = carry + ex;
        carry += tot;
    }
    if (threadIdx.x == 0) *grand = carry;
}

template <typename TIn>
__global__ __launch_bounds__(SCAN_THREADS) void k_tile_scan(const TIn *in, long long n, const long long *tile_off,
                                                            long long *out) {
    __shared__ long long smem[4];
    long long base = (long long)blockIdx.x * SCAN_TILE + (long long)threadIdx.x * SCAN_ITEMS;
    long long v[SCAN_ITEMS];
    long long s = 0;
#pragma unroll
    for (int k = 0; k < SCAN_ITEMS; k++) {
        v[k] = (base + k < n) ? (long long)in[base + k] : 0;
        s += v[k];
    }
    long long tot;
    long long ex = block_exclusive_scan(s, &tot, smem) + tile_off[blockIdx.x];
#pragma unroll
    for (int k = 0; k < SCAN_ITEMS; k++) {
        if (base + k < n) out[base + k] = ex;
        ex += v[k];
    }
}

template <typename TIn>
static int exclusive_scan(hipStream_t st, const TIn *in, int64_t *out, int64_t n, int64_t *h_total) {
    XM_ARG(n >= 0);
    XM_SCOPE(st);
    int64_t n_tiles = (n + SCAN_TILE - 1) / SCAN_TILE;
    long long *tile = nullptr;
    XM_HIP(xm_malloc_async((void **)&tile, sizeof(long long) * (size_t)(n_tiles + 1), st));
    if (n_tiles > 0) {
        k_tile_sums<TIn><<<dim3((unsigned)n_tiles), dim3(SCAN_THREADS), 0, st>>>(in, n, tile);
        XM_LAUNCH_CHECK();
    }
    k_scan_tile_sums<<<dim3(1), dim3(SCAN_THREADS), 0, st>>>(tile, n_tiles, (long long *)(out + n));
    XM_LAUNCH_CHECK();
    if (n_tiles > 0) {
        k_tile_scan<TIn><<<dim3((unsigned)n_tiles), dim3(SCAN_THREADS), 0, st>>>(in, n, tile, (long long *)out);
        XM_LAUNCH_CHECK();
    }
    XM_HIP(xm_free_async(tile, st));
    if (h_total) {
        XM_HIP(hipMemcpyAsync(h_total, out + n, sizeof(int64_t), hipMemcpyDeviceToHost, st));
        XM_HIP(hipStreamSynchronize(st));
    }
    return XMAP_OK;
}
}

extern "C" {
const char *xmap_last_error(void) { return xmap::g_err; }
int xmap_version(void) { return 101; }

int xmap_trim(void) {
    XM_HIP(hipDeviceSynchronize());
    int dev = 0;
    XM_HIP(hipGetDevice(&dev));
    for (xmap::Arena &a : xmap::g_arenas) {
        if (a.dev != dev || a.live != 0) continue;
        for (xmap::Chunk &c : a.chunks) (void)hipFree(c.base);
        a.chunks.clear();
    }
    return XMAP_OK;
}

int xmap_debug_arena(void *stream, int64_t *live, int64_t *reserved) {
    XM_ARG(live && reserved);
    int dev = 0;
    XM_HIP(hipGetDevice(&dev));
    *live = 0; *reserved = 0;
    if (xmap::Arena *a = xmap::arena_find(dev, (hipStream_t)stream)) {
        *live = (int64_t)a->live;
        for (xmap::Chunk &c : a->chunks) *reserved += (int64_t)c.size;
    }
    return XMAP_OK;
}
int xmap_debug_arena_call(void *stream, int64_t bytes, int fail) {
    using namespace xmap;
    XM_SCOPE(stream);
    hipStream_t st = (hipStream_t)stream;
    void *a = nullptr, *b = nullptr;
    XM_HIP(xm_malloc_async(&a, (size_t)bytes, st));
    XM_HIP(xm_malloc_async(&b, 1024, st));
    XM_ARG(!fail);
    XM_HIP(xm_free_async(b, st));
    XM_HIP(xm_free_async(a, st));
    return XMAP_OK;
}

int xmap_exclusive_scan_i64(void *stream, const int64_t *in, int64_t *out, int64_t n, int64_t *h_total) {
    return xmap::exclusive_scan<long long>((hipStream_t)stream, (const long long *)in, out, n, h_total);
}
int xmap_exclusive_scan_i32_to_i64(void *stream, const int32_t *in, int64_t *out, int64_t n, int64_t *h_total) {
    return xmap::exclusive_scan<int>((hipStream_t)stream, in, out, n, h_total);
}
}
```

x-map_amd/xmap/engine/device.py:

```python
import ctypes as C
import os

import numpy as np
import torch

from . import hipabi as abi
from .exactness import plain_sums_exact

lib = abi.lib
vp, i32, i64, check = abi.vp, abi.i32, abi.i64, abi.check


def _stream(dev):
    return C.c_void_p(torch.cuda.current_stream(dev).cuda_stream)


SLOT_TARGET = 768
CH_MIN = 2048


class DeviceRatings(object):

    def __init__(self, user_ptr, item, rating, time, n_items, attrs, device="cuda:0", rating64=False):
        self.device = torch.device(device)
# ... 276 lines not shown
                raise abi.XmapError(abi.ERR_OVERFLOW, "pair-table overflow")
            break
        kept, evaluated = int(h_cnt[0]), int(h_cnt[1])
        unit_off = self._zeros(nu + 1, torch.int64)
        check(lib.xmap_exclusive_scan_i32_to_i64(st, vp(unit_cnt), vp(unit_off), i64(nu), None))
        row_ptr = self._empty(I + 1, torch.int64)
        abi.xcheck(abi.xlib().xmap_sim_row_ptr(st, i32(I), vp(unit_ptr), vp(unit_off), vp(row_ptr)))
        col = self._empty(max(kept, 1), torch.int32)
        sim = self._empty(max(kept, 1), torch.float64)
        mutu = self._empty(max(kept, 1), torch.int32)
        nij = self._empty(max(kept, 1), torch.int32)
        with self.timed("pair_fill"):
            abi.xcheck(abi.xlib().xmap_sim_fill(st, C.byref(R.c), m, int(cap), vp(u_avg), vp(info), vp(ua_item), vp(ia_user),
                                    vp(Q), vp(unit_item), vp(unit_q), i64(lo), i64(hi), vp(unit_off),
                                    vp(col), vp(sim), vp(mutu), vp(nij)))
        S = SimResult()
        S.method, S.cap, S.n_items = abi.METHODS[method] if isinstance(method, str) else int(method), int(cap), I
        S.u_avg, S.u_norm, S.info = u_avg, u_norm, info
        S.row_ptr, S.col, S.sim, S.mutu, S.nij = row_ptr, col[:kept], sim[:kept], mutu[:kept], nij[:kept]
        S.n_kept, S.n_eval, S.n_contrib, S.n_units = kept, evaluated, int(contrib), hi - lo
        S.plan = Pn
        S.slot_target = slot_target
        S.c = abi.Sim(I, row_ptr.data_ptr(), col.data_ptr(), sim.data_ptr(), mutu.data_ptr(), nij.data_ptr(),
                      info.data_ptr(), 0)
        S._keep = (col, sim, mutu, nij)
        return S

    def tri_layout(self, stats, slot_target=SLOT_TARGET, ch_min=CH_MIN, dups=False):
        R = self.R
        st = _stream(self.dev)
        I, U, nnz = R.n_items, R.n_users, R.nnz
        info = stats[2]
        L = SimResult()
        L.hist = self._empty(U + 2, torch.int32)
        L.pre = self._empty(U + 3, torch.int64)
        L.ctl = self._empty(4, torch.int32)
        L.hid = self._empty(max(I, 1), torch.int32)
        L.hlist = self._zeros(1024, torch.int32)
        L.ub_key = self._empty(max(nnz, 1), torch.int64)
        L.ub = self._empty(max(nnz, 1), torch.int64)
        L.rc = self._empty(max(nnz, 1) * 2, torch.int64)
        L.Wp = self._empty(max(I, 1), torch.int64)
        L.dups = bool(dups)
        h_ctl = (C.c_int32 * 2)()
        with self.timed("tri_layout"):
            check(lib.xmap_sim2_layout(st, C.byref(R.c), vp(info), i32(ch_min), vp(L.hist), vp(L.pre), vp(L.ctl),
                                       vp(L.hid), vp(L.hlist), vp(L.ub_key), vp(L.ub), vp(L.rc), vp(L.Wp),
                                       i32(1 if dups else 0), h_ctl))
        L.CH, L.n_heavy = int(h_ctl[0]), int(h_ctl[1])
        L.slot_target = slot_target
        self._tri_plan(L, slot_target)
        both = torch.stack([L.Wp[:I].sum(), L.Wp[L.hlist[:L.n_heavy].long()].sum()]).tolist() if I else [0, 0]
        L.half_contrib, L.heavy_half = int(both[0]), int(both[1])
        return L

    def _tri_plan(self, L, slot_target):
        R = self.R
        st = _stream(self.dev)
        I = R.n_items
        L.Q = self._out(max(I, 1), torch.int32, I > 0)
        L.C = self._out(max(I, 1), torch.int32, I > 0)
        L.small = self._out(max(I, 1), torch.uint8, I > 0)
        L.Qcat = self._empty(5 * max(I, 1), torch.int32)
        L.uq_ptr = self._out(5 * I + 1, torch.int64, I > 0)
        L.uc_ptr = self._out(I + 1, torch.int64, I > 0)
        h = (C.c_int64 * 8)()
        with self.timed("tri_plan"):
            check(lib.xmap_sim2_plan(st, C.byref(R.c), i32(slot_target), vp(L.rc), vp(L.pre), vp(L.hid),
                                     vp(L.ctl), vp(L.Q), vp(L.C), vp(L.small), vp(L.Wp), vp(L.Qcat), vp(L.uq_ptr),
                                     vp(L.uc_ptr), i32(1 if getattr(L, "dups", False) else 0), h))
            L.n_light, L.n_heavy_units = int(h[0]), int(h[1])
            L.cls_ptr = (C.c_int64 * 6)(*[int(h[2 + c]) for c in range(6)])
            L.uq_item = self._empty(max(L.n_light, 1), torch.int32)
            L.uq_q = self._empty(4 * max(L.n_light, 1), torch.int32)
            L.uc_item = self._empty(max(L.n_heavy_units, 1), torch.int32)
            L.uc_c = self._empty(max(L.n_heavy_units, 1), torch.int32)
            check(lib.xmap_sim2_units(st, i32(I), vp(R.item_ptr), vp(L.Qcat), vp(L.uq_ptr), vp(L.uq_item), vp(L.uq_q),
                                      vp(L.C), vp(L.uc_ptr), vp(L.uc_item), vp(L.uc_c)))
        L.slot_target = slot_target

    def _tri_plan3(self, L, slot_target):
        R = self.R
        st = _stream(self.dev)
        I = R.n_items
        L.Q = self._out(max(I, 1), torch.int32, I > 0)
        L.C = self._out(max(I, 1), torch.int32, I > 0)
        L.small = self._out(max(I, 1), torch.uint8, I > 0)
        L.Qcat = self._empty(5 * max(I, 1), torch.int32)
        L.uq_ptr = self._out(5 * I + 1, torch.int64, I > 0)
        L.uc_ptr = self._out(I + 1, torch.int64, I > 0)
        cap_light = L.half_contrib // max(int(slot_target), 1) + I + 1
        cap_heavy = R.nnz // max(int(L.ch_min), 1) + 1025
        L.uq_item = self._empty(cap_light, torch.int32)
        L.uq_q = self._empty(4 * cap_light, torch.int32)
        L.uc_item = self._empty(cap_heavy, torch.int32)
        L.uc_c = self._empty(cap_heavy, torch.int32)
        h = (C.c_int64 * 10)()
        with self.timed("tri_plan"):
            check(lib.xmap_sim3_plan(st, C.byref(R.c), i32(slot_target), vp(L.pre), vp(L.hid), vp(L.ctl), vp(L.Q), vp(L.C),
                                     vp(L.small), vp(L.Wp), vp(L.Qcat), vp(L.uq_ptr), vp(L.uc_ptr),
                                     i32(1 if getattr(L, "dups", False) else 0), vp(L.uq_item), vp(L.uq_q), vp(L.uc_item),
                                     vp(L.uc_c), i64(cap_light), i64(cap_heavy), h))
        L.n_light, L.n_heavy_units = int(h[0]), int(h[1])
        L.cls_ptr = (C.c_int64 * 6)(*[int(h[2 + c]) for c in range(6)])
        L.CH, L.n_heavy = int(h[8]), int(h[9])
        L.slot_target = slot_target
        L.replan = self._tri_plan3

    def heavy_half(self, L):
        if getattr(L, "_heavy_half", None) is None:
            L._heavy_half = int(L.Wp[L.hlist[:L.n_heavy].long()].sum().item()) if L.n_heavy else 0
        return L._heavy_half

    def tri_pairs(self, method, cap, stats, L, unit_range=None, do_heavy=True, retry=True, rec=False, raw=False, split=False,
                  heavy_deal=None, marks=True, count_mir=False):
        R = self.R
        st = _stream(self.dev)
        m = self.pair_method(method)
        u_avg, u_norm, info, _, _ = stats
        I = R.n_items
        coo_slack = 1.0
        while True:
            lo, hi = (0, L.n_light) if unit_range is None else (int(unit_range[0]), int(unit_range[1]))
            cap_coo = (max(int(L.half_contrib * coo_slack), 1) // 4096 + 1100) * 4096
            coo_i = self._empty(cap_coo, torch.int32)
            coo_j = self._empty(cap_coo, torch.int32)
            coo_sim = self._empty(cap_coo, torch.float64)
            coo_mutu = self._empty(cap_coo, torch.int32)
            coo_nij = self._empty(cap_coo, torch.int32)
            coo_ls = self._empty(cap_coo, torch.float64) if (rec or raw) else None
            rowcnt = self._empty(max(I, 1), torch.int32)
            mircnt = self._empty(max(I, 1), torch.int32) if split else None
            nh = L.n_heavy_units if do_heavy else 0
            hp_hi = self._empty(max(nh, 1) * 1024, torch.float64)
            hp_lo = self._empty(max(nh, 1) * 1024, torch.float64)
            hp_cnt = self._empty(max(nh, 1) * 1024, torch.int32)
            hp_mut = self._empty(max(nh, 1) * 1024, torch.int32)
            d_cnt = self._zeros(6, torch.int64)
            d_shards = self._empty(2 * 4096, torch.int64)
            rowcnt_h = self._empty(64 * 1024, torch.int32)

            deal = 0 if heavy_deal is None else ((int(heavy_deal[1]) & 0xff) << 16) | ((int(heavy_deal[0]) & 0xff) << 8)

            def run(phases):
                phases |= deal | (0 if marks else 128)
                check(lib.xmap_sim2_pairs(
                    st, C.byref(R.c), m, int(cap), vp(u_avg), vp(self.norms), vp(L.rc), vp(L.ub), vp(L.Q), vp(L.small),
                    vp(L.uq_item),
                    vp(L.uq_q), L.cls_ptr, i64(lo), i64(hi), vp(L.hid), vp(L.hlist), vp(L.ctl), vp(L.C), vp(L.uc_ptr),
                    vp(L.uc_item), vp(L.uc_c), i32(nh), i32(L.n_heavy), phases,
                    vp(hp_hi), vp(hp_lo), vp(hp_cnt), vp(hp_mut), i64(cap_coo), vp(coo_i), vp(coo_j), vp(coo_sim),
                    vp(coo_mutu), vp(coo_nij), vp(coo_ls), vp(rowcnt), vp(rowcnt_h), vp(d_shards), vp(d_cnt), vp(mircnt)))
            if os.environ.get("XMAP_SPLIT_PHASES") == "1":
                with self.timed("pair_heavy"):
                    run(8 | (1 if do_heavy else 0))
                with self.timed("pair_tri"):
                    run(2 | (32 if raw else 0))
                with self.timed("heavy_merge"):
                    run((4 if do_heavy else 0) | 16)
            else:
                with self.timed("pair_tri"):
                    run(8 | 2 | 16 | 64 | (5 if do_heavy else 0) | (32 if raw else 0))
            if count_mir and split and not raw:
                with self.timed("mir_count"):
                    scratch = self._empty(cap_coo, torch.int32)
                    check(lib.xmap_sim3_mircount(st, i32(I), i64(cap_coo), vp(coo_i), vp(coo_j), vp(d_shards), i64(cap_coo),
                                                 i32(1 if rec else 0), vp(scratch), vp(mircnt)))
            h = d_cnt.tolist()
            if h[2]:
                if L.slot_target <= 32:
                    raise abi.XmapError(abi.ERR_OVERFLOW, "pair-table overflow")
                if not retry:
                    return (None, rowcnt, 0, 0) + ((None, None) if split else ()) + (1,)
                getattr(L, "replan", self._tri_plan)(L, L.slot_target // 2)
                continue
            if h[3]:
                if coo_slack > 64:
                    raise abi.XmapError(abi.ERR_CAPACITY, "half-COO overflow")
                coo_slack *= 2
                continue
            break
        if os.environ.get("XMAP_SPLIT_PHASES") == "1":
            h[4:6] = d_shards.view(2, 4096).sum(dim=1).tolist()
        n, n_unordered = int(h[4]), int(h[5])
        coo = (coo_i, coo_j, coo_sim, coo_mutu, coo_nij) + ((coo_ls,) if (rec or raw) else ())
        out = (coo, rowcnt, n, n_unordered)
        if split:
            return out + (mircnt, d_shards) + (() if retry else (0,))
        return out if retry else out + (0,)

    def tri_scatter(self, coo, rowcnt, info, n=None, L=None):
        R = self.R
        st = _stream(self.dev)
        I = R.n_items
        coo_i, coo_j, coo_sim, coo_mutu, coo_nij = [x.contiguous() for x in coo[:5]]
        coo_ls = coo[5].contiguous() if len(coo) > 5 else None
        n_scan = int(coo_i.numel())
        if n is None:
            n = n_scan
        row_ptr = self._out(I + 1, torch.int64, I > 0)
        tot = C.c_int64(0)
        check(lib.xmap_exclusive_scan_i32_to_i64(st, vp(rowcnt), vp(row_ptr), i64(I), C.byref(tot) if coo_ls is not None else None))
        kept = 2 * n if coo_ls is None else int(tot.value)
        ls = self._empty(max(kept, 1), torch.float64) if coo_ls is not None else None
        col = self._empty(max(kept, 1), torch.int32)
        sim = self._empty(max(kept, 1), torch.float64)
        mutu = self._empty(max(kept, 1), torch.int32)
        nij = self._empty(max(kept, 1), torch.int32)
        fill = self._empty(max(I, 1), torch.int32)
        with self.timed("scatter"):
          if n:
            check(lib.xmap_sim2_scatter(st, i32(I), i64(n_scan), vp(coo_i), vp(coo_j), vp(coo_sim), vp(coo_mutu),
                                        vp(coo_nij), vp(coo_ls), vp(row_ptr), vp(fill), vp(L.hid), vp(L.hlist), vp(col),
                                        vp(sim), vp(mutu), vp(nij), vp(ls)))
        S = self.sim_from_device(row_ptr, col[:kept], sim[:kept], mutu[:kept], nij[:kept], info)
        S.ls = ls[:kept] if ls is not None else None
        return S

    def rec_sim(self, cap, slot_target=SLOT_TARGET):
        R = self.R
        with self.timed("rec_stats"):
            stats, L = self.layout3(slot_target, ch_min=max(64, R.n_users + 2), wide=True)
        info = stats[2]
        if os.environ.get("XMAP_A_V2") == "1":
            coo, rowcnt, n, n_unordered = self.tri_pairs("adjust_cosine", cap, stats, L, do_heavy=False, rec=True)
            S = self.tri_scatter(coo, rowcnt, info, n, L)
        else:
            coo, own, n, n_unordered, mir, shards = self.tri_pairs("adjust_cosine", cap, stats, L, do_heavy=False, rec=True, split=True, marks=False, count_mir=True)
            S = self.tri_mirror(coo, own, mir, info, n, shards, counted=True)
        S.cap, S.n_unordered, S.layout = int(cap), n_unordered, L
        S.norm = self.norms[R.n_items:2 * R.n_items]
        return S

    def rec_select(self, S, keep):
        st = _stream(self.dev)
        I = self.R.n_items
        cnt = self._zeros(max(I, 1), torch.int32)
        col = self._empty((max(I, 1), keep), torch.int32)
        sim = self._empty((max(I, 1), keep), torch.float64)
        ls = self._empty((max(I, 1), keep), torch.float64)
        with self.timed("rec_select"):
            check(lib.xmap_rec_select(st, i32(I), vp(S.row_ptr), vp(S.col), vp(S.sim), vp(S.ls), i32(keep), vp(cnt),
                                      vp(col), vp(sim), vp(ls)))
        return cnt[:I], col[:I], sim[:I], ls[:I]

    def layout3(self, slot_target=SLOT_TARGET, ch_min=CH_MIN, wide=False, item_range=None):
        R = self.R
        st = _stream(self.dev)
        I, U, nnz = R.n_items, R.n_users, R.nnz
        n1, i1 = max(nnz, 1), max(I, 1)
        rw = 3 if wide else 2
        L = SimResult()
        cnt = self._empty(i1, torch.int32)
        u_avg = self._zeros(max(U, 1), torch.float64) if wide else self._empty(max(U, 1), torch.float64)
        u_norm = None if wide else self._empty(max(U, 1), torch.float64)
        L.hist = self._empty(U + 2, torch.int32)
        L.pre = self._empty(U + 3, torch.int64)
        L.ctl = self._empty(4, torch.int32)
        L.hid = self._empty(i1, torch.int32)
        L.hlist = self._zeros(1024, torch.int32)
        L.ub_key = self._empty(n1, torch.int64)
        L.ub = self._empty(n1 * (2 if wide else 1), torch.int64)
        srec = self._empty(n1 * rw, torch.int64)
        buf_a = self._empty(n1 * rw, torch.int64)
        buf_b = self._empty(n1 * rw, torch.int64)
        L.rc = self._empty(n1 * 2, torch.int64)
        L.Wp = self._empty(i1, torch.int64)
        L.dups = bool(wide)
        L.wide = bool(wide)
        info = self._out((i1, 4), torch.float64, I > 0)
        self.norms = self._out(2 * i1, torch.float64, I > 0)
        r64 = None
        if wide:
            r64 = R.user_rating64 if R.user_rating64 is not None else R.user_rating.double()
        def call(phases, lo, hi):
            check(lib.xmap_sim3_layout(st, C.byref(R.c), vp(R.item_ptr), vp(r64), i32(ch_min), i32(phases), i32(lo), i32(hi), vp(cnt),
                                       vp(u_avg), vp(u_norm), vp(L.hist), vp(L.pre), vp(L.ctl), vp(L.hid), vp(L.hlist),
                                       vp(L.ub_key), vp(L.ub), vp(srec), vp(buf_a), vp(buf_b), vp(L.rc), vp(L.Wp), vp(info),
                                       vp(self.norms), None))
        R.csc_ready = False
        L.ch_min = int(ch_min)
        L.half_contrib = R.half_contrib
        if item_range is None:
            with self.timed("layout3"):
                call(1 | 2 | 4, 0, I)
            self._tri_plan3(L, slot_target)
        else:
            with self.timed("layout3"):
                call(1 | 2, int(item_range[0]), int(item_range[1]))

            def finish():
                with self.timed("layout3_flags"):
                    call(4 | 8, 0, I)
                self._tri_plan3(L, slot_target)
            L.finish = finish
        return (u_avg, u_norm, info, None, None), L

    def mir_counts(self, coo, n, mir, shards=None, skip_self=False):
        I = self.R.n_items
        scratch = self._empty(max(int(n), 1), torch.int32)
        check(lib.xmap_sim3_mircount(_stream(self.dev), i32(I), i64(int(coo[0].numel())), vp(coo[0].contiguous()), vp(coo[1].contiguous()),
                                     vp(shards), i64(n), i32(1 if skip_self else 0), vp(scratch), vp(mir)))
        return mir

    def tri_mirror(self, coo, own, mir, info, n, shards=None, rows=None, counted=False):
        R = self.R
        st = _stream(self.dev)
        I = R.n_items
        coo_i, coo_j, coo_sim, coo_mutu, coo_nij = [x.contiguous() for x in coo[:5]]
        coo_ls = coo[5].contiguous() if len(coo) > 5 else None
        cap = int(coo_i.numel())
        kept = 2 * int(n)
        lo, hi = (0, I) if rows is None else (int(rows[0]), int(rows[1]))
        if rows is not None and I > 0:
            own = own.clone()
            own[:lo].zero_(); own[hi:].zero_()
            if counted:
                mir = mir.clone()
                mir[:lo].zero_(); mir[hi:].zero_()
                kept = int((own[lo:hi].long().sum() + mir[lo:hi].long().sum()).item())
        rw = 4 if coo_ls is not None else 3
        row_ptr = self._out(I + 1, torch.int64, I > 0)
        mptr = self._empty(I + 1, torch.int64)
        tot = self._empty(max(I, 1), torch.int32)
        fill = self._empty(max(I, 1), torch.int32)
        buf_a = self._empty(max(int(n), 1) * rw, torch.int64)
        buf_b = self._empty(max(int(n), 1) * rw, torch.int64)
        col = self._empty(max(kept, 1), torch.int32)
        sim = self._empty(max(kept, 1), torch.float64)
        mutu = self._empty(max(kept, 1), torch.int32)
        nij = self._empty(max(kept, 1), torch.int32)
        ls = self._empty(max(kept, 1), torch.float64) if coo_ls is not None else None
        with self.timed("scatter"):
            if not counted:
                check(lib.xmap_sim3_mircount(st, i32(I), i64(cap), vp(coo_i), vp(coo_j), vp(shards), i64(n), i32(1 if coo_ls is not None else 0),
                                             vp(buf_a), vp(mir)))
                if rows is not None and I > 0:
                    mir[:lo].zero_(); mir[hi:].zero_()
                    kept = int((own[lo:hi].long().sum() + mir[lo:hi].long().sum()).item())
            check(lib.xmap_sim3_mirror(st, i32(I), i64(cap), vp(coo_i), vp(coo_j), vp(coo_sim), vp(coo_mutu), vp(coo_nij), vp(shards), i64(n),
                                       vp(own), vp(mir), vp(tot), vp(row_ptr), vp(mptr), vp(fill), vp(buf_a), vp(buf_b), vp(col),
                                       vp(sim), vp(mutu), vp(nij), vp(coo_ls), vp(ls), i32(lo), i32(hi)))
        if coo_ls is not None:
            kept = int(row_ptr[I].item()) if I > 0 else 0
        S = self.sim_from_device(row_ptr, col[:kept], sim[:kept], mutu[:kept], nij[:kept], info)
        S.ls = ls[:kept] if ls is not None else None
        return S

    def item_sim_tri(self, method, cap, slot_target=SLOT_TARGET, ch_min=CH_MIN):
        if os.environ.get("XMAP_A_V2") == "1":
            with self.timed("stats"):
                stats = self.stats()
            L = self.tri_layout(stats, slot_target, ch_min)
            coo, rowcnt, n, n_unordered = self.tri_pairs(method, cap, stats, L)
            S = self.tri_scatter(coo, rowcnt, stats[2], n, L)
        else:
            stats, L = self.layout3(slot_target, ch_min)
            coo, rowcnt, n, n_unordered, mir, shards = self.tri_pairs(method, cap, stats, L, split=True, marks=False, count_mir=True)
            S = self.tri_mirror(coo, rowcnt, mir, stats[2], n, shards, counted=True)
        S.method = abi.METHODS[method] if isinstance(method, str) else int(method)
        S.cap = int(cap)
        S.u_avg, S.u_norm = stats[0], stats[1]
        S.n_eval, S.n_contrib = 2 * n_unordered, 2 * L.half_contrib
        S.n_units, S.layout, S.slot_target = L.n_light + L.n_heavy_units, L, L.slot_target
        return S

    def sim_from_device(self, row_ptr, col, sim, mutu, nij, info):
        S = SimResult()
        S.n_items = self.R.n_items
        n = int(col.numel())
        if n == 0:
            col = self._zeros(1, torch.int32); sim = self._zeros(1, torch.float64)
            mutu = self._zeros(1, torch.int32); nij = self._zeros(1, torch.int32)
        S.row_ptr, S.info = row_ptr.contiguous(), info
        col, sim, mutu, nij = col.contiguous(), sim.contiguous(), mutu.contiguous(), nij.contiguous()
        S.col, S.sim, S.mutu, S.nij = col[:n], sim[:n], mutu[:n], nij[:n]
        S.n_kept = n
        S.c = abi.Sim(S.n_items, S.row_ptr.data_ptr(), col.data_ptr(), sim.data_ptr(), mutu.data_ptr(),
                      nij.data_ptr(), info.data_ptr())
        S._keep = (col, sim, mutu, nij)
        return S

    def sim_from_host(self, row_ptr, col, sim, mutu, nij, info, frac=None):
        d = self.dev
        n = int(row_ptr[-1])

        def up(a, dt):
            return torch.from_numpy(np.ascontiguousarray(a if n else np.zeros(1), dt)).to(d)
        row_ptr_d = torch.from_numpy(np.ascontiguousarray(row_ptr, np.int64)).to(d)
        info_d = torch.from_numpy(np.ascontiguousarray(info, np.float64)).to(d)
        S = self.sim_from_device(row_ptr_d, up(col, np.int32)[:n], up(sim, np.float64)[:n], up(mutu, np.int32)[:n],
                                 up(nij if nij is not None else np.zeros(max(n, 1)), np.int32)[:n], info_d)
        if frac is not None:
            S.frac = up(frac, np.float64)
            S.c.frac = S.frac.data_ptr()
        return S

    def knn(self, S, top_k, bb=None, rows=None):
        R = self.R
        st = _stream(self.dev)
        I, k = R.n_items, int(top_k)
        E = ExtResult()
        E.k = k
        if bb is not None:
            E.bb = bb.to(torch.uint8).contiguous()
        else:
            E.bb = self._zeros(max(I, 1), torch.uint8)
            check(lib.xmap_bridge_flags(st, C.byref(S.c), vp(R.prefix_cls), vp(E.bb)))
        alloc = self._empty if I > 0 else self._zeros
        E.cls = alloc(max(I, 1), torch.uint8)
        E.kcnt = alloc((max(I, 1), 2), torch.int32)
        E.kcol = alloc((max(I, 1), 2, k), torch.int32)
        E.kval = alloc((max(I, 1), 2, k, 3), torch.float64)
        with self.timed("knn_classify"):
            lo, hi = (0, I) if rows is None else (int(rows[0]), int(rows[1]))
            check(lib.xmap_knn_classify(st, C.byref(S.c), k, vp(E.bb), vp(R.suffix_cls), vp(R.contains_mask),
                                        vp(E.cls), vp(E.kcnt), vp(E.kcol), vp(E.kval), i32(lo), i32(hi)))
        return E

    def _reverse(self, S, E, mode, attach_ptr):
        st8 = self.reverse_count(S, E, mode, attach_ptr, None)
        self.reverse_fill(st8)
        return st8.out

    def reverse_count(self, S, E, mode, attach_ptr, rows):
        R = self.R
        I = R.n_items
        st8 = ExtResult()
        st8.S, st8.E, st8.mode = S, E, mode
        st8.rows = (0, I) if rows is None else (int(rows[0]), int(rows[1]))
        st8.rcnt = self._zeros(max(I, 1), torch.int32)
        st8.eflag = self._empty(max(int(S.col.numel()), 1), torch.uint8)
        st8.args = (C.byref(S.c), mode, E.k, vp(E.bb), vp(E.cls), vp(E.kcnt), vp(E.kcol), vp(E.kval),
                    vp(R.suffix_cls), vp(R.contains_mask), vp(R.flags), vp(attach_ptr), vp(getattr(E, "thr", None)),
                    vp(getattr(E, "long_rows", None)), vp(st8.eflag))
        st8.keep = attach_ptr
        check(lib.xmap_reverse_count(_stream(self.dev), *st8.args, vp(st8.rcnt), i32(st8.rows[0]), i32(st8.rows[1])))
        return st8

    def reverse_count_pair(self, S, E, rows):
        R = self.R
        I = R.n_items
# ... 620 lines not shown
```

x-map_amd/xmap/engine/hipabi.py:

```python
import ctypes as C
import os

HERE = os.path.dirname(os.path.abspath(__file__))
LIB_PATH = os.environ.get("XMAP_HIP_LIB") or os.path.normpath(os.path.join(HERE, "..", "..", "libxmap_hip.so"))
XLIB_PATH = os.environ.get("XMAP_HIP_XLIB") or os.path.normpath(os.path.join(HERE, "..", "..", "libxmap_hip_xcheck.so"))

COSINE, ADJUST_COSINE = 0, 1
METHODS = {"cosine": COSINE, "adjust_cosine": ADJUST_COSINE}
COSINE_EXACT = 2
TOPC = 10
MID_ROWS_SPAN = 36864
ERR_HIP, ERR_ARG, ERR_OVERFLOW, ERR_CAPACITY = -1, -2, -3, -4


class XmapError(RuntimeError):
    def __init__(self, code, msg):
        RuntimeError.__init__(self, "libxmap_hip error %d: %s" % (code, msg))
        self.code = code


class Ratings(C.Structure):
    _fields_ = [("n_users", C.c_int64), ("n_items", C.c_int32), ("nnz", C.c_int64),
                ("user_ptr", C.c_void_p), ("user_item", C.c_void_p), ("user_rating", C.c_void_p),
                ("user_time", C.c_void_p), ("item_ptr", C.c_void_p), ("item_user", C.c_void_p),
                ("item_rating", C.c_void_p), ("prefix_cls", C.c_void_p), ("suffix_cls", C.c_void_p),
                ("contains_mask", C.c_void_p), ("flags", C.c_void_p)]


class Sim(C.Structure):
    _fields_ = [("n_items", C.c_int32), ("row_ptr", C.c_void_p), ("col", C.c_void_p), ("sim", C.c_void_p),
                ("mutu", C.c_void_p), ("nij", C.c_void_p), ("info", C.c_void_p), ("frac", C.c_void_p)]


class ExtTables(C.Structure):
    _fields_ = [("n_items", C.c_int32), ("top_k", C.c_int32),
                ("cls", C.c_void_p), ("kcnt", C.c_void_p), ("kcol", C.c_void_p), ("kval", C.c_void_p), ("flags", C.c_void_p),
                ("att_ptr", C.c_void_p), ("att_idx", C.c_void_p), ("att_val", C.c_void_p),
                ("src_ptr", C.c_void_p), ("src_idx", C.c_void_p), ("src_val", C.c_void_p), ("src_flag", C.c_void_p),
                ("rnn_ptr", C.c_void_p), ("rnn_idx", C.c_void_p), ("rnn_val", C.c_void_p),
                ("n_nb", C.c_int32), ("nb_id", C.c_void_p), ("nb_list", C.c_void_p), ("midX", C.c_void_p), ("dir", C.c_void_p),
                ("dir_ptr", C.c_void_p),
                ("n_ends", C.c_int32), ("urank", C.c_void_p), ("uitem", C.c_void_p)]


class PathUnits(C.Structure):
    _fields_ = [("n_units", C.c_int32), ("unit_start", C.c_void_p), ("unit_c", C.c_void_p), ("unit_G", C.c_void_p),
                ("unit_row", C.c_void_p), ("unit_nt", C.c_void_p), ("n_heavy", C.c_int32), ("heavy_unit0", C.c_void_p)]


class PathRows(C.Structure):
    _fields_ = [("n_slots", C.c_int32), ("acc", C.c_void_p), ("touched", C.c_void_p), ("hacc", C.c_void_p),
                ("htouched", C.c_void_p)]


class PathOut(C.Structure):
    _fields_ = [("n_cand", C.c_void_p), ("top_end", C.c_void_p), ("top_val", C.c_void_p), ("xs_cap", C.c_int64),
                ("xs_off", C.c_void_p), ("xs_end", C.c_void_p), ("xs_val", C.c_void_p)]


EXPORTS = [
    "xmap_last_error", "xmap_version", "xmap_trim", "xmap_debug_arena", "xmap_debug_arena_call", "xmap_exclusive_scan_i64", "xmap_exclusive_scan_i32_to_i64",
    "xmap_build_csc", "xmap_user_stats", "xmap_item_stats", 
    "xmap_sim2_layout", "xmap_sim2_plan", "xmap_sim2_units",
    "xmap_sim2_pairs", "xmap_sim2_scatter", "xmap_sim3_layout", "xmap_sim3_plan", "xmap_sim3_mircount", "xmap_sim3_mirror", "xmap_item_partials", "xmap_item_merge", "xmap_sim2_pack_partials",
    "xmap_sim2_sort_partials", "xmap_sim2_merge_partials", "xmap_sim2_pack_pairs", "xmap_sim2_unpack_pairs", "xmap_bridge_flags", "xmap_knn_classify", "xmap_knn_thresholds", "xmap_reverse_count", "xmap_reverse_count_att_rnn",
    "xmap_reverse_fill", "xmap_topc_from_lists", "xmap_path_weights", "xmap_extend_paths", 
    "xmap_mid_rows_count", "xmap_mid_rows_place", "xmap_edge_ranges", "xmap_end_universe", "xmap_extend_cols", "xmap_extend_cols_slots", "xmap_nb_index", "xmap_path_plan", "xmap_end_order", "xmap_dense_normalize", "xmap_dense_layout", "xmap_dense_topk", "xmap_rec_select", "xmap_predict", "xmap_rec_profiles", "xmap_predict_rows", "xmap_mae", "xmap_select_map", "xmap_alterego_count", "xmap_alterego_fill",
    "xmap_feed_text", "xmap_feed_texts", "xmap_feed_merge", "xmap_feed_sizes", "xmap_feed_arrays", "xmap_feed_ids", "xmap_feed_free",
    "xmap_ctx_upload_feed", "xmap_feed_format", "xmap_ctx_create", "xmap_ctx_destroy", "xmap_ctx_upload_ratings", "xmap_ctx_item_sim", "xmap_ctx_sim_download", "xmap_ctx_extend",
    "xmap_ctx_ext_download", "xmap_ctx_ext_lists", "xmap_ctx_candidates", "xmap_ctx_generate", "xmap_ctx_gen_download",
    "xmap_ctx_rec_sim", "xmap_ctx_rec_profiles_download", "xmap_ctx_rec_download", "xmap_ctx_rec_select", "xmap_ctx_rec_set_neighbors",
    "xmap_ctx_rec_neighbors_download", "xmap_ctx_predict",
]

if not os.path.exists(LIB_PATH):
    raise ImportError("libxmap_hip.so not built (%s); the MI355X engine has no CPU fallback" % LIB_PATH)
lib = C.CDLL(LIB_PATH)
lib.xmap_last_error.restype = C.c_char_p
for _n in EXPORTS:
    getattr(lib, _n)
XCHECK_EXPORTS = ["xmap_sim_plan", "xmap_sim_units", "xmap_sim_count", "xmap_sim_fill", "xmap_sim_row_ptr", "xmap_extend_paths2",
                  "xmap_mid_tally", "xmap_mid_place"]

HEADER_PATH = os.path.normpath(os.path.join(HERE, "..", "..", "..", "include", "xmap_hip.h"))


def header_prototypes(path=HEADER_PATH):
    import re
    with open(path) as f:
        text = f.read()
    text = re.sub(r"#\s*ifdef\s+XMAP_CROSSCHECK[^\n]*\n", "\n", text)
    text = re.sub(r"/\*.*?\*/", " ", text, flags=re.S)
    text = re.sub(r"//[^\n]*", " ", text)
    out = {}
    for m in re.finditer(r"\b(?:int|void|const\s+char\s*\*)\s*(xmap_\w+)\s*\(([^;{]*?)\)\s*;", text, flags=re.S):
        name, args = m.group(1), " ".join(m.group(2).split())
        types = []
        for a in ([] if args in ("", "void") else args.split(",")):
            if "*" in a:
                types.append(C.c_void_p)
            elif "int64_t" in a:
                types.append(C.c_int64)
            elif "double" in a:
                types.append(C.c_double)
            elif "float" in a:
                types.append(C.c_float)
            else:
                types.append(C.c_int32)
        out[name] = types
    return out


PROTOTYPES = header_prototypes()


def _bind(L, names):
    for _n in names:
        _f = getattr(L, _n)
        _f.argtypes = PROTOTYPES[_n]
        if _n in ("xmap_ctx_destroy", "xmap_feed_free"):
            _f.restype = None
        elif _n != "xmap_last_error":
            _f.restype = C.c_int


_bind(lib, [n for n in PROTOTYPES if n not in XCHECK_EXPORTS])
_xlib = None


def xlib():
    global _xlib
    if _xlib is None:
        if not os.path.exists(XLIB_PATH):
            raise ImportError("libxmap_hip_xcheck.so not built (%s): make -C x-map_amd/csrc" % XLIB_PATH)
        L = C.CDLL(XLIB_PATH)
        L.xmap_last_error.restype = C.c_char_p
        _bind(L, list(PROTOTYPES))
        _xlib = L
    return _xlib


def check(rc):
    if rc != 0:
        raise XmapError(rc, (lib.xmap_last_error() or b"").decode())
# ... 20 lines not shown
```

Measured before the change: 23.15 billion.

## Fuse layout and plan stages and overlap host readback with mirror counting

Measured after the change: 23.14 billion. No clear change (-0.0%).

```diff
diff --git a/include/xmap_hip.h b/include/xmap_hip.h
--- a/include/xmap_hip.h
+++ b/include/xmap_hip.h
@@ -44,6 +44,9 @@
 
 int xmap_exclusive_scan_i64(void *stream, const int64_t *in, int64_t *out, int64_t n, int64_t *h_total);
 int xmap_exclusive_scan_i32_to_i64(void *stream, const int32_t *in, int64_t *out, int64_t n, int64_t *h_total);
+
+int xmap_host_post(void *stream, const int64_t *d_words, int32_t n_words, int32_t *ticket );
+int xmap_host_wait(int32_t ticket, int64_t *h_words , int32_t n_words);
 
 
 int xmap_build_csc(void *stream, int64_t n_users, int32_t n_items, int64_t nnz, const int64_t *user_ptr,
@@ -117,6 +120,12 @@
                    const int32_t *ctl, int32_t *Q, int32_t *C, uint8_t *small, uint64_t *Wp, int32_t *Qcat ,
                    int64_t *uq_ptr , int64_t *uc_ptr , int32_t dups, int32_t *uq_item, int32_t *uq_q ,
                    int32_t *uc_item, int32_t *uc_c, int64_t cap_light, int64_t cap_heavy, int64_t *h_out );
+int xmap_sim4_layout_plan(void *stream, const xmap_ratings *R, int64_t *item_ptr, const double *rating64, int32_t ch_min, int32_t *cnt,
+                          double *u_avg, double *u_norm, int32_t *hist, int64_t *pre, int32_t *ctl, int32_t *hid, int32_t *hlist,
+                          uint64_t *ub_key, void *ub, void *srec, void *bufA, void *bufB, void *rc, uint64_t *Wp, double *info,
+                          double *norms, int32_t slot_target, int32_t *Q, int32_t *C, uint8_t *small, int32_t *Qcat, int64_t *uq_ptr,
+                          int64_t *uc_ptr, int32_t dups, int32_t *uq_item, int32_t *uq_q, int32_t *uc_item, int32_t *uc_c,
+                          int64_t cap_light, int64_t cap_heavy, int64_t *h_out );
 int xmap_sim3_mircount(void *stream, int32_t n_items, int64_t coo_cap, const int32_t *coo_i, const int32_t *coo_j,
                        const int64_t *d_shards , int64_t n_pairs, int32_t skip_self, void *scratch, int32_t *mir );
 int xmap_sim3_mirror(void *stream, int32_t n_items, int64_t coo_cap, const int32_t *coo_i, const int32_t *coo_j,
diff --git a/x-map_amd/csrc/api.hip b/x-map_amd/csrc/api.hip
--- a/x-map_amd/csrc/api.hip
+++ b/x-map_amd/csrc/api.hip
@@ -283,8 +283,6 @@
     T_ALLOC(ub_key, n1); T_ALLOC(ub, n1); T_ALLOC(rcrec, 2 * n1); T_ALLOC(Wp, I);
     T_ALLOC(srec, 2 * n1); T_ALLOC(buf_a, 2 * n1); T_ALLOC(buf_b, 2 * n1);
     const int ch_min = 2048;
-    XM_TRY(xmap_sim3_layout(c->st, &R, (int64_t *)R.item_ptr, nullptr, ch_min, 1 | 2 | 4, 0, I, cnt, c->u_avg, c->u_norm, hist, pre, ctl,
-                            hid, hlist, ub_key, ub, srec, buf_a, buf_b, rcrec, Wp, c->info, norms, nullptr));
     const int64_t half_contrib = c->half_contrib;
     int32_t *Q, *Cc, *Qcat, *uq_item = nullptr, *uq_q = nullptr, *uc_item = nullptr, *uc_c = nullptr;
     uint8_t *small;
@@ -296,16 +294,21 @@
     int64_t hc[10];
     int64_t n_light = 0, n_hu = 0;
     int n_heavy = 0;
-    auto plan = [&](int target) -> int {
+    auto plan = [&](int target, bool first) -> int {
         const int64_t cap_light = half_contrib / target + I + 1, cap_heavy = nnz / ch_min + 1025;
         T_ALLOC(uq_item, cap_light); T_ALLOC(uq_q, 4 * cap_light); T_ALLOC(uc_item, cap_heavy); T_ALLOC(uc_c, cap_heavy);
-        XM_TRY(xmap_sim3_plan(c->st, &R, target, pre, hid, ctl, Q, Cc, small, Wp, Qcat, uq_ptr, uc_ptr, 0, uq_item, uq_q, uc_item, uc_c,
-                              cap_light, cap_heavy, hc));
+        if (first)
+            XM_TRY(xmap_sim4_layout_plan(c->st, &R, (int64_t *)R.item_ptr, nullptr, ch_min, cnt, c->u_avg, c->u_norm, hist, pre, ctl, hid,
+                                         hlist, ub_key, ub, srec, buf_a, buf_b, rcrec, Wp, c->info, norms, target, Q, Cc, small, Qcat,
+                                         uq_ptr, uc_ptr, 0, uq_item, uq_q, uc_item, uc_c, cap_light, cap_heavy, hc));
+        else
+            XM_TRY(xmap_sim3_plan(c->st, &R, target, pre, hid, ctl, Q, Cc, small, Wp, Qcat, uq_ptr, uc_ptr, 0, uq_item, uq_q, uc_item, uc_c,
+                                  cap_light, cap_heavy, hc));
         n_light = hc[0]; n_hu = hc[1]; n_heavy = (int)hc[9];
         return XMAP_OK;
     };
-    XM_TRY(plan(slot_target));
-    int32_t *coo_i = nullptr, *coo_j = nullptr, *coo_mutu = nullptr, *coo_nij = nullptr, *own = nullptr, *mir = nullptr;
+    XM_TRY(plan(slot_target, true));
+    int32_t *coo_i = nullptr, *coo_j = nullptr, *coo_mutu = nullptr, *coo_nij = nullptr, *own = nullptr, *mir = nullptr, *mir_part = nullptr;
     double *coo_sim = nullptr;
     int64_t *d_shards = nullptr;
     int64_t cap_coo = 0, n = 0, n_unordered = 0;
@@ -315,7 +318,7 @@
         int32_t *hp_cnt, *hp_mut, *rowcnt_h;
         int64_t *d_cnt;
         T_ALLOC(coo_i, cap_coo); T_ALLOC(coo_j, cap_coo); T_ALLOC(coo_sim, cap_coo); T_ALLOC(coo_mutu, cap_coo); T_ALLOC(coo_nij, cap_coo);
-        T_ALLOC(own, I); T_ALLOC(mir, I);
+        T_ALLOC(own, I); T_ALLOC(mir, I); T_ALLOC(mir_part, cap_coo);
         const size_t hp = (size_t)(n_hu ? n_hu : 1) * 1024;
         T_ALLOC(hp_hi, hp); T_ALLOC(hp_lo, hp); T_ALLOC(hp_cnt, hp); T_ALLOC(hp_mut, hp);
         T_ALLOCZ(d_cnt, 6); T_ALLOC(d_shards, 2 * 4096); T_ALLOC(rowcnt_h, 64 * 1024);
@@ -323,12 +326,14 @@
                                ctl, Cc, uc_ptr, uc_item, uc_c, (int32_t)n_hu, n_heavy, 8 | 1 | 2 | 4 | 16 | 64 | 128, hp_hi, hp_lo, hp_cnt,
                                hp_mut, cap_coo, coo_i, coo_j, coo_sim, coo_mutu, coo_nij, nullptr, own, rowcnt_h, d_shards, d_cnt, mir));
         int64_t h_cnt[6];
-        XM_TRY(d2h(h_cnt, d_cnt, 6, c->st));
-        XM_HIP(hipStreamSynchronize(c->st));
+        int32_t ticket = -1;
+        XM_TRY(xmap_host_post(c->st, d_cnt, 6, &ticket));
+        XM_TRY(xmap_sim3_mircount(c->st, I, cap_coo, coo_i, coo_j, d_shards, cap_coo, 0, mir_part, mir));
+        XM_TRY(xmap_host_wait(ticket, h_cnt, 6));
         if (h_cnt[2]) {
             if (slot_target <= 32) { set_error("pair-table overflow"); return XMAP_ERR_OVERFLOW; }
             slot_target /= 2;
-            XM_TRY(plan(slot_target));
+            XM_TRY(plan(slot_target, false));
             continue;
         }
         if (h_cnt[3]) {
@@ -348,7 +353,6 @@
     uint64_t *mir_a, *mir_b;
     XM_ALLOC(c->p_sim, col, kept); XM_ALLOC(c->p_sim, sim, kept); XM_ALLOC(c->p_sim, mutu, kept); XM_ALLOC(c->p_sim, nij, kept);
     T_ALLOC(fill, I); T_ALLOC(tot, I); T_ALLOC(mir_a, (size_t)3 * (n ? n : 1)); T_ALLOC(mir_b, (size_t)3 * (n ? n : 1));
-    XM_TRY(xmap_sim3_mircount(c->st, I, cap_coo, coo_i, coo_j, d_shards, n, 0, mir_a, mir));
     XM_TRY(xmap_sim3_mirror(c->st, I, cap_coo, coo_i, coo_j, coo_sim, coo_mutu, coo_nij, d_shards, n, own, mir, tot, row_ptr, mptr, fill,
                             mir_a, mir_b, col, sim, mutu, nij, nullptr, nullptr, 0, I));
     XM_HIP(hipStreamSynchronize(c->st));
@@ -622,8 +626,6 @@
     T_ALLOC(ub_key, n1); T_ALLOC(ub, 2 * n1); T_ALLOC(rcrec, 2 * n1); T_ALLOC(Wp, i1);
     T_ALLOC(srec, 3 * n1); T_ALLOC(buf_a, 3 * n1); T_ALLOC(buf_b, 3 * n1);
     const int ch_min = (int)((U + 2 > 64) ? U + 2 : 64);
-    XM_TRY(xmap_sim3_layout(c->st, &P, item_ptr, c->pf_rating, ch_min, 1 | 2 | 4, 0, I, cnt, u_avg, nullptr, hist, pre, ctl, hid, hlist,
-                            ub_key, ub, srec, buf_a, buf_b, rcrec, Wp, info, norms, nullptr));
     int32_t *Q, *Cc, *Qcat, *uq_item = nullptr, *uq_q = nullptr, *uc_item = nullptr, *uc_c = nullptr;
     uint8_t *small;
     int64_t *uq_ptr, *uc_ptr;
@@ -633,16 +635,21 @@
     double coo_slack = 1.0;
     int64_t hc[10];
     int64_t n_light = 0;
-    auto plan = [&](int target) -> int {
+    auto plan = [&](int target, bool first) -> int {
         const int64_t cap_light = half_contrib / target + I + 1, cap_heavy = nnz / ch_min + 1025;
         T_ALLOC(uq_item, cap_light); T_ALLOC(uq_q, 4 * cap_light); T_ALLOC(uc_item, cap_heavy); T_ALLOC(uc_c, cap_heavy);
-        XM_TRY(xmap_sim3_plan(c->st, &P, target, pre, hid, ctl, Q, Cc, small, Wp, Qcat, uq_ptr, uc_ptr, 1, uq_item, uq_q, uc_item, uc_c,
-                              cap_light, cap_heavy, hc));
+        if (first)
+            XM_TRY(xmap_sim4_layout_plan(c->st, &P, item_ptr, c->pf_rating, ch_min, cnt, u_avg, nullptr, hist, pre, ctl, hid, hlist, ub_key,
+                                         ub, srec, buf_a, buf_b, rcrec, Wp, info, norms, target, Q, Cc, small, Qcat, uq_ptr, uc_ptr, 1,
+                                         uq_item, uq_q, uc_item, uc_c, cap_light, cap_heavy, hc));
+        else
+            XM_TRY(xmap_sim3_plan(c->st, &P, target, pre, hid, ctl, Q, Cc, small, Wp, Qcat, uq_ptr, uc_ptr, 1, uq_item, uq_q, uc_item, uc_c,
+                                  cap_light, cap_heavy, hc));
         n_light = hc[0];
         return XMAP_OK;
     };
-    XM_TRY(plan(slot_target));
-    int32_t *coo_i = nullptr, *coo_j = nullptr, *coo_mutu = nullptr, *coo_nij = nullptr, *own = nullptr, *mir = nullptr;
+    XM_TRY(plan(slot_target, true));
+    int32_t *coo_i = nullptr, *coo_j = nullptr, *coo_mutu = nullptr, *coo_nij = nullptr, *own = nullptr, *mir = nullptr, *mir_part = nullptr;
     double *coo_sim = nullptr, *coo_ls = nullptr;
     int64_t *d_shards = nullptr;
     int64_t cap_coo = 0, n = 0;
@@ -652,19 +659,21 @@
         int32_t *hp_cnt, *hp_mut, *rowcnt_h;
         int64_t *d_cnt;
         T_ALLOC(coo_i, cap_coo); T_ALLOC(coo_j, cap_coo); T_ALLOC(coo_sim, cap_coo); T_ALLOC(coo_mutu, cap_coo); T_ALLOC(coo_nij, cap_coo);
-        T_ALLOC(coo_ls, cap_coo); T_ALLOC(own, i1); T_ALLOC(mir, i1);
+        T_ALLOC(coo_ls, cap_coo); T_ALLOC(own, i1); T_ALLOC(mir, i1); T_ALLOC(mir_part, cap_coo);
         T_ALLOC(hp_hi, 1024); T_ALLOC(hp_lo, 1024); T_ALLOC(hp_cnt, 1024); T_ALLOC(hp_mut, 1024);
         T_ALLOCZ(d_cnt, 6); T_ALLOC(d_shards, 2 * 4096); T_ALLOC(rowcnt_h, 64 * 1024);
         XM_TRY(xmap_sim2_pairs(c->st, &P, XMAP_ADJUST_COSINE, cap, u_avg, norms, rcrec, ub, Q, small, uq_item, uq_q, hc + 2, 0, n_light, hid,
                                hlist, ctl, Cc, uc_ptr, uc_item, uc_c, 0, 0, 8 | 2 | 16 | 64 | 128, hp_hi, hp_lo, hp_cnt, hp_mut, cap_coo,
                                coo_i, coo_j, coo_sim, coo_mutu, coo_nij, coo_ls, own, rowcnt_h, d_shards, d_cnt, mir));
         int64_t h_cnt[6];
-        XM_TRY(d2h(h_cnt, d_cnt, 6, c->st));
-        XM_HIP(hipStreamSynchronize(c->st));
+        int32_t ticket = -1;
+        XM_TRY(xmap_host_post(c->st, d_cnt, 6, &ticket));
+        XM_TRY(xmap_sim3_mircount(c->st, I, cap_coo, coo_i, coo_j, d_shards, cap_coo, 1, mir_part, mir));
+        XM_TRY(xmap_host_wait(ticket, h_cnt, 6));
         if (h_cnt[2]) {
             if (slot_target <= 32) { set_error("pair-table overflow"); return XMAP_ERR_OVERFLOW; }
             slot_target /= 2;
-            XM_TRY(plan(slot_target));
+            XM_TRY(plan(slot_target, false));
             continue;
         }
         if (h_cnt[3]) {
@@ -683,7 +692,6 @@
     XM_ALLOC(c->p_rec, c->rs_col, kept_max); XM_ALLOC(c->p_rec, c->rs_sim, kept_max); XM_ALLOC(c->p_rec, c->rs_nij, kept_max);
     XM_ALLOC(c->p_rec, c->rs_ls, kept_max);
     T_ALLOC(mutu, kept_max); T_ALLOC(fill, i1); T_ALLOC(tot, i1); T_ALLOC(mir_a, 4 * nn); T_ALLOC(mir_b, 4 * nn);
-    XM_TRY(xmap_sim3_mircount(c->st, I, cap_coo, coo_i, coo_j, d_shards, n, 1, mir_a, mir));
     XM_TRY(xmap_sim3_mirror(c->st, I, cap_coo, coo_i, coo_j, coo_sim, coo_mutu, coo_nij, d_shards, n, own, mir, tot, c->rs_row_ptr, mptr, fill,
                             mir_a, mir_b, c->rs_col, c->rs_sim, mutu, c->rs_nij, coo_ls, c->rs_ls, 0, I));
     XM_HIP(hipMemcpy2DAsync(c->rs_avg, sizeof(double), info, 4 * sizeof(double), sizeof(double), (size_t)I, hipMemcpyDeviceToDevice, c->st));
diff --git a/x-map_amd/csrc/common.h b/x-map_amd/csrc/common.h
--- a/x-map_amd/csrc/common.h
+++ b/x-map_amd/csrc/common.h
@@ -42,6 +42,10 @@
     XmScope &operator=(const XmScope &) = delete;
 };
 #define XM_SCOPE(stream) xmap::XmScope xm_scope_((hipStream_t)(stream))
+constexpr size_t XM_HOST_SLOT_BYTES = 128;
+int host_post(hipStream_t st, const void *d_src, size_t bytes, int *ticket);
+int host_wait(int ticket, void *dst, size_t bytes);
+int exclusive_scan2_i32(hipStream_t st, const int32_t *a, const int32_t *b, int64_t n, int32_t *ab, int64_t *out_ab, int64_t *out_b);
 int radix_sort_pairs(hipStream_t st, unsigned long long *keys, int *vals, unsigned long long *keys_tmp, int *vals_tmp, long long n,
                      int bits);
 
diff --git a/x-map_amd/csrc/stage_a2.hip b/x-map_amd/csrc/stage_a2.hip
--- a/x-map_amd/csrc/stage_a2.hip
+++ b/x-map_amd/csrc/stage_a2.hip
@@ -1029,7 +1029,7 @@
 
 template <bool SELF>
 __global__ __launch_bounds__(CB_T) void k_cbs_hist(long long range_cap, int n_ranges, const unsigned long long *cur, const int *coo_i,
-                                                   const int *coo_j, int sh, unsigned *bcnt) {
+                                                   const int *coo_j, int sh, int n_items, unsigned *bcnt) {
     __shared__ unsigned h[CB_MAX];
     for (int t = threadIdx.x; t < CB_MAX; t += CB_T) h[t] = 0u;
     __syncthreads();
@@ -1047,7 +1047,7 @@
             const long long e = c * CB_CHUNK + q * CB_T + threadIdx.x;
             if (e < n) {
                 const int j = coo_j[b + e];
-                if (!SELF || j != coo_i[b + e]) atomicAdd(&h[j >> sh], 1u);
+                if ((unsigned)j < (unsigned)n_items && (!SELF || j != coo_i[b + e])) atomicAdd(&h[j >> sh], 1u);
             }
         }
     }
@@ -1058,7 +1058,7 @@
 
 template <bool SELF>
 __global__ __launch_bounds__(CB_T) void k_cbs_scatter(long long range_cap, int n_ranges, const unsigned long long *cur, const int *coo_i,
-                                                      const int *coo_j, int sh, const long long *bptr, unsigned *bcur, int *out) {
+                                                      const int *coo_j, int sh, int n_items, const long long *bptr, unsigned *bcur, int *out) {
     static_assert(CB_T == CB_MAX, "one thread per bucket in the scan");
     __shared__ unsigned h[CB_MAX], off[CB_MAX + 1], wsum[CB_T / 64];
     __shared__ long long base[CB_MAX];
@@ -1083,7 +1083,7 @@
             it[sg][q] = -1;
             if (e < n) {
                 const int j = coo_j[b + e];
-                if (!SELF || j != coo_i[b + e]) it[sg][q] = j;
+                if ((unsigned)j < (unsigned)n_items && (!SELF || j != coo_i[b + e])) it[sg][q] = j;
             }
         }
     }
@@ -1721,18 +1721,79 @@
     XM_HIP(hipMemsetAsync(bcnt, 0, sizeof(unsigned) * CB_MAX, st));
     const long long segs = (long long)n_ranges * ((range_cap + CB_CHUNK - 1) / CB_CHUNK);
     const dim3 g((unsigned)((segs + CB_SPB - 1) / CB_SPB));
-    if (skip_self) k_cbs_hist<true><<<g, dim3(CB_T), 0, st>>>(range_cap, n_ranges, cur, coo_i, coo_j, sh, bcnt);
-    else k_cbs_hist<false><<<g, dim3(CB_T), 0, st>>>(range_cap, n_ranges, cur, coo_i, coo_j, sh, bcnt);
+    if (skip_self) k_cbs_hist<true><<<g, dim3(CB_T), 0, st>>>(range_cap, n_ranges, cur, coo_i, coo_j, sh, n_items, bcnt);
+    else k_cbs_hist<false><<<g, dim3(CB_T), 0, st>>>(range_cap, n_ranges, cur, coo_i, coo_j, sh, n_items, bcnt);
     XM_LAUNCH_CHECK();
     k_cb_scan<<<dim3(1), dim3(CB_MAX), 0, st>>>(bcnt, bptr, bcur);
     XM_LAUNCH_CHECK();
-    if (skip_self) k_cbs_scatter<true><<<g, dim3(CB_T), 0, st>>>(range_cap, n_ranges, cur, coo_i, coo_j, sh, bptr, bcur, part);
-    else k_cbs_scatter<false><<<g, dim3(CB_T), 0, st>>>(range_cap, n_ranges, cur, coo_i, coo_j, sh, bptr, bcur, part);
+    if (skip_self) k_cbs_scatter<true><<<g, dim3(CB_T), 0, st>>>(range_cap, n_ranges, cur, coo_i, coo_j, sh, n_items, bptr, bcur, part);
+    else k_cbs_scatter<false><<<g, dim3(CB_T), 0, st>>>(range_cap, n_ranges, cur, coo_i, coo_j, sh, n_items, bptr, bcur, part);
     XM_LAUNCH_CHECK();
     const long long cap = range_cap * n_ranges;
     k_cb_count<<<dim3((unsigned)((cap + (long long)CB_CHUNK * CB_SPB - 1) / ((long long)CB_CHUNK * CB_SPB))), dim3(CB_T), 0, st>>>(
         -1, part, sh, bptr, n_items, counts);
     XM_LAUNCH_CHECK();
+    return XMAP_OK;
+}
+}
+
+namespace {
+__global__ void k_plan_words(int I, const long long *uq_ptr, const long long *uc_ptr, const int *ctl, long long *out) {
+    const int t = threadIdx.x;
+    if (t >= 10) return;
+    long long v = 0;
+    if (t >= 8) v = ctl[t - 8];
+    else if (I > 0) v = t == 0 ? uq_ptr[(long long)N_CLASSES * I] : t == 1 ? uc_ptr[I] : uq_ptr[(long long)(t - 2) * I];
+    out[t] = v;
+}
+
+int plan3_enqueue(hipStream_t st, const xmap_ratings *R, int32_t slot_target, const int64_t *pre, const int32_t *hid, const int32_t *ctl,
+                  int32_t *Q, int32_t *C, uint8_t *small, uint64_t *Wp, int32_t *Qcat, int64_t *uq_ptr, int64_t *uc_ptr, int32_t dups,
+                  int32_t *uq_item, int32_t *uq_q, int32_t *uc_item, int32_t *uc_c, int64_t cap_light, int64_t cap_heavy, int64_t *h_out,
+                  int *ticket) {
+    XM_ARG(R && Wp && pre && hid && ctl && Q && C && small && Qcat && uq_ptr && uc_ptr && h_out);
+    XM_ARG(uq_item && uq_q && uc_item && uc_c && cap_light >= 0 && cap_heavy >= 0);
+    XM_ARG(slot_target > 0 && slot_target <= T_SLOTS);
+    const int I = R->n_items;
+    for (int c = 0; c < 10; c++) h_out[c] = 0;
+    XM_HIP(hipMemsetAsync(Qcat, 0, sizeof(int32_t) * (size_t)N_CLASSES * (size_t)(I > 0 ? I : 1), st));
+    if (I > 0) {
+        k_plan2<<<dim3((unsigned)((I + 255) / 256)), dim3(256), 0, st>>>(
+            I, (const long long *)R->item_ptr, nullptr, (const long long *)pre, (int)R->n_users + 2, hid, ctl, slot_target, dups, Q, C,
+            small, (unsigned long long *)Wp, Qcat);
+        XM_LAUNCH_CHECK();
+    }
+    int rcode = xmap_exclusive_scan_i32_to_i64(st, Qcat, uq_ptr, (int64_t)N_CLASSES * I, nullptr);
+    if (rcode) return rcode;
+    rcode = xmap_exclusive_scan_i32_to_i64(st, C, uc_ptr, I, nullptr);
+    if (rcode) return rcode;
+    if (I > 0) {
+        k_fill_units2<<<dim3((unsigned)(((long long)N_CLASSES * I + 255) / 256)), dim3(256), 0, st>>>(
+            I, (const long long *)R->item_ptr, Qcat, (const long long *)uq_ptr, uq_item, uq_q, C, (const long long *)uc_ptr, uc_item, uc_c,
+            cap_light, cap_heavy);
+        XM_LAUNCH_CHECK();
+    }
+    long long *words = nullptr;
+    XM_HIP(xm_malloc_async((void **)&words, 10 * sizeof(long long), st));
+    k_plan_words<<<dim3(1), dim3(64), 0, st>>>(I, (const long long *)uq_ptr, (const long long *)uc_ptr, ctl, words);
+    XM_LAUNCH_CHECK();
+    rcode = host_post(st, words, 10 * sizeof(long long), ticket);
+    if (rcode) return rcode;
+    XM_HIP(xm_free_async(words, st));
+    return XMAP_OK;
+}
+int plan3_finish(int ticket, int64_t cap_light, int64_t cap_heavy, int64_t *h_out) {
+    int rcode = host_wait(ticket, h_out, 10 * sizeof(int64_t));
+    if (rcode) return rcode;
+    if (h_out[9] > HMAX) {
+        set_error("heavy set larger than %d", HMAX);
+        return XMAP_ERR_OVERFLOW;
+    }
+    if (h_out[0] > cap_light || h_out[1] > cap_heavy) {
+        set_error("unit arrays too small: %lld light / %lld heavy units, room for %lld / %lld", (long long)h_out[0], (long long)h_out[1],
+                  (long long)cap_light, (long long)cap_heavy);
+        return XMAP_ERR_CAPACITY;
+    }
     return XMAP_OK;
 }
 }
@@ -1837,47 +1898,33 @@
                    int64_t *uc_ptr, int32_t dups, int32_t *uq_item, int32_t *uq_q, int32_t *uc_item, int32_t *uc_c,
                    int64_t cap_light, int64_t cap_heavy, int64_t *h_out) {
     XM_SCOPE(stream);
-    XM_ARG(R && Wp && pre && hid && ctl && Q && C && small && Qcat && uq_ptr && uc_ptr && h_out);
-    XM_ARG(uq_item && uq_q && uc_item && uc_c && cap_light >= 0 && cap_heavy >= 0);
-    XM_ARG(slot_target > 0 && slot_target <= T_SLOTS);
-    hipStream_t st = (hipStream_t)stream;
+    int ticket = -1;
+    int rcode = plan3_enqueue((hipStream_t)stream, R, slot_target, pre, hid, ctl, Q, C, small, Wp, Qcat, uq_ptr, uc_ptr, dups, uq_item, uq_q,
+                              uc_item, uc_c, cap_light, cap_heavy, h_out, &ticket);
+    if (rcode) return rcode;
+    return plan3_finish(ticket, cap_light, cap_heavy, h_out);
+}
+
+int xmap_sim4_layout_plan(void *stream, const xmap_ratings *R, int64_t *item_ptr, const double *rating64, int32_t ch_min, int32_t *cnt,
+                          double *u_avg, double *u_norm, int32_t *hist, int64_t *pre, int32_t *ctl, int32_t *hid, int32_t *hlist,
+                          uint64_t *ub_key, void *ub, void *srec, void *bufA, void *bufB, void *rc, uint64_t *Wp, double *info,
+                          double *norms, int32_t slot_target, int32_t *Q, int32_t *C, uint8_t *small, int32_t *Qcat, int64_t *uq_ptr,
+                          int64_t *uc_ptr, int32_t dups, int32_t *uq_item, int32_t *uq_q, int32_t *uc_item, int32_t *uc_c,
+                          int64_t cap_light, int64_t cap_heavy, int64_t *h_out) {
+    XM_SCOPE(stream);
+    XM_ARG(R);
     const int I = R->n_items;
-    for (int c = 0; c < 10; c++) h_out[c] = 0;
-    XM_HIP(hipMemsetAsync(Qcat, 0, sizeof(int32_t) * (size_t)N_CLASSES * (size_t)(I > 0 ? I : 1), st));
-    if (I > 0) {
-        k_plan2<<<dim3((unsigned)((I + 255) / 256)), dim3(256), 0, st>>>(
-            I, (const long long *)R->item_ptr, nullptr, (const long long *)pre, (int)R->n_users + 2, hid, ctl, slot_target, dups, Q, C,
-            small, (unsigned long long *)Wp, Qcat);
-        XM_LAUNCH_CHECK();
-    }
-    int rcode = xmap_exclusive_scan_i32_to_i64(stream, Qcat, uq_ptr, (int64_t)N_CLASSES * I, nullptr);
+    int rcode = xmap_sim3_layout(stream, R, item_ptr, rating64, ch_min, 1, 0, I, cnt, u_avg, u_norm, hist, pre, ctl, hid, hlist, ub_key, ub,
+                                 srec, bufA, bufB, rc, Wp, info, norms, nullptr);
     if (rcode) return rcode;
-    rcode = xmap_exclusive_scan_i32_to_i64(stream, C, uc_ptr, I, nullptr);
+    int ticket = -1;
+    rcode = plan3_enqueue((hipStream_t)stream, R, slot_target, pre, hid, ctl, Q, C, small, Wp, Qcat, uq_ptr, uc_ptr, dups, uq_item, uq_q,
+                          uc_item, uc_c, cap_light, cap_heavy, h_out, &ticket);
     if (rcode) return rcode;
-    if (I > 0) {
-        k_fill_units2<<<dim3((unsigned)(((long long)N_CLASSES * I + 255) / 256)), dim3(256), 0, st>>>(
-            I, (const long long *)R->item_ptr, Qcat, (const long long *)uq_ptr, uq_item, uq_q, C, (const long long *)uc_ptr, uc_item, uc_c,
-            cap_light, cap_heavy);
-        XM_LAUNCH_CHECK();
-        XM_HIP(hipMemcpy2DAsync(&h_out[2], sizeof(int64_t), uq_ptr, sizeof(int64_t) * (size_t)I, sizeof(int64_t), N_CLASSES + 1,
-                                hipMemcpyDeviceToHost, st));
-        XM_HIP(hipMemcpyAsync(&h_out[1], uc_ptr + I, sizeof(int64_t), hipMemcpyDeviceToHost, st));
-    }
-    int32_t h_ctl[2] = {0, 0};
-    XM_HIP(hipMemcpyAsync(h_ctl, ctl, 2 * sizeof(int32_t), hipMemcpyDeviceToHost, st));
-    XM_HIP(hipStreamSynchronize(st));
-    h_out[0] = h_out[2 + N_CLASSES];
-    h_out[8] = h_ctl[0]; h_out[9] = h_ctl[1];
-    if (h_ctl[1] > HMAX) {
-        set_error("heavy set larger than %d", HMAX);
-        return XMAP_ERR_OVERFLOW;
-    }
-    if (h_out[0] > cap_light || h_out[1] > cap_heavy) {
-        set_error("unit arrays too small: %lld light / %lld heavy units, room for %lld / %lld", (long long)h_out[0], (long long)h_out[1],
-                  (long long)cap_light, (long long)cap_heavy);
-        return XMAP_ERR_CAPACITY;
-    }
-    return XMAP_OK;
+    rcode = xmap_sim3_layout(stream, R, item_ptr, rating64, ch_min, 2 | 4, 0, I, cnt, u_avg, u_norm, hist, pre, ctl, hid, hlist, ub_key, ub,
+                             srec, bufA, bufB, rc, Wp, info, norms, nullptr);
+    if (rcode) return rcode;
+    return plan3_finish(ticket, cap_light, cap_heavy, h_out);
 }
 
 int xmap_sim2_pairs(void *stream, const xmap_ratings *R, int method, int cap, const double *u_avg, const double *norms,
@@ -2306,13 +2353,16 @@
     XM_ARG((coo_aux != nullptr) == (aux != nullptr));
     hipStream_t st = (hipStream_t)stream;
     const int I = n_items;
-    if (I > 0) {
-        k_row_totals<<<dim3((unsigned)((I + 255) / 256)), dim3(256), 0, st>>>(I, own, mir, tot);
-        XM_LAUNCH_CHECK();
-    }
-    int rcode = xmap_exclusive_scan_i32_to_i64(stream, tot, row_ptr, I, nullptr);
-    if (rcode) return rcode;
-    rcode = xmap_exclusive_scan_i32_to_i64(stream, mir, mptr, I, nullptr);
+    int rcode = exclusive_scan2_i32(st, own, mir, I, tot, row_ptr, mptr);
+    if (rcode == XMAP_ERR_CAPACITY) {
+        if (I > 0) {
+            k_row_totals<<<dim3((unsigned)((I + 255) / 256)), dim3(256), 0, st>>>(I, own, mir, tot);
+            XM_LAUNCH_CHECK();
+        }
+        rcode = xmap_exclusive_scan_i32_to_i64(stream, tot, row_ptr, I, nullptr);
+        if (rcode) return rcode;
+        rcode = xmap_exclusive_scan_i32_to_i64(stream, mir, mptr, I, nullptr);
+    }
     if (rcode) return rcode;
     if (n_pairs == 0 || I == 0 || coo_cap == 0) return XMAP_OK;
     XM_HIP(hipMemsetAsync(fill, 0, sizeof(int32_t) * (size_t)I, st));
diff --git a/x-map_amd/csrc/util.hip b/x-map_amd/csrc/util.hip
--- a/x-map_amd/csrc/util.hip
+++ b/x-map_amd/csrc/util.hip
@@ -1,5 +1,6 @@
 #include <stdarg.h>
 #include <stdlib.h>
+#include <string.h>
 #include <vector>
 
 #include "common.h"
@@ -159,6 +160,88 @@
     }
 }
 
+constexpr int SCAN_SELF_MAX = 2048;
+template <typename TIn>
+__global__ __launch_bounds__(SCAN_THREADS) void k_tile_scan_self(const TIn *in, long long n, const long long *tile_sum, long long *out) {
+    __shared__ long long smem[4];
+    long long part = 0;
+    for (int i = threadIdx.x; i < (int)blockIdx.x; i += SCAN_THREADS) part += tile_sum[i];
+    long long off;
+    block_exclusive_scan(part, &off, smem);
+    long long base = (long long)blockIdx.x * SCAN_TILE + (long long)threadIdx.x * SCAN_ITEMS;
+    long long v[SCAN_ITEMS];
+    long long s = 0;
+#pragma unroll
+    for (int k = 0; k < SCAN_ITEMS; k++) {
+        v[k] = (base + k < n) ? (long long)in[base + k] : 0;
+        s += v[k];
+    }
+    long long tot;
+    long long ex = block_exclusive_scan(s, &tot, smem) + off;
+#pragma unroll
+    for (int k = 0; k < SCAN_ITEMS; k++) {
+        if (base + k < n) out[base + k] = ex;
+        ex += v[k];
+    }
+    if (blockIdx.x == gridDim.x - 1 && threadIdx.x == 0) out[n] = off + tot;
+}
+
+__global__ __launch_bounds__(SCAN_THREADS) void k_tile_sums2(const int *a, const int *b, long long n, long long *tile_sum ) {
+    __shared__ long long smem[4];
+    long long base = (long long)blockIdx.x * SCAN_TILE + (long long)threadIdx.x * SCAN_ITEMS;
+    long long sa = 0, sb = 0;
+#pragma unroll
+    for (int k = 0; k < SCAN_ITEMS; k++)
+        if (base + k < n) { sa += (long long)a[base + k]; sb += (long long)b[base + k]; }
+    long long ta, tb;
+    block_exclusive_scan(sa + sb, &ta, smem);
+    block_exclusive_scan(sb, &tb, smem);
+    if (threadIdx.x == 0) { tile_sum[blockIdx.x] = ta; tile_sum[gridDim.x + blockIdx.x] = tb; }
+}
+__global__ __launch_bounds__(SCAN_THREADS) void k_tile_scan2_self(const int *a, const int *b, long long n, const long long *tile_sum,
+                                                                  int *ab, long long *out_ab, long long *out_b) {
+    __shared__ long long smem[4];
+    long long pa = 0, pb = 0;
+    for (int i = threadIdx.x; i < (int)blockIdx.x; i += SCAN_THREADS) { pa += tile_sum[i]; pb += tile_sum[gridDim.x + i]; }
+    long long off_a, off_b;
+    block_exclusive_scan(pa, &off_a, smem);
+    block_exclusive_scan(pb, &off_b, smem);
+    long long base = (long long)blockIdx.x * SCAN_TILE + (long long)threadIdx.x * SCAN_ITEMS;
+    long long va[SCAN_ITEMS], vb[SCAN_ITEMS];
+    long long sa = 0, sb = 0;
+#pragma unroll
+    for (int k = 0; k < SCAN_ITEMS; k++) {
+        const bool in = base + k < n;
+        vb[k] = in ? (long long)b[base + k] : 0;
+        va[k] = (in ? (long long)a[base + k] : 0) + vb[k];
+        sa += va[k]; sb += vb[k];
+    }
+    long long ta, tb;
+    long long ea = block_exclusive_scan(sa, &ta, smem) + off_a;
+    long long eb = block_exclusive_scan(sb, &tb, smem) + off_b;
+#pragma unroll
+    for (int k = 0; k < SCAN_ITEMS; k++) {
+        if (base + k < n) { ab[base + k] = (int)va[k]; out_ab[base + k] = ea; out_b[base + k] = eb; }
+        ea += va[k]; eb += vb[k];
+    }
+    if (blockIdx.x == gridDim.x - 1 && threadIdx.x == 0) { out_ab[n] = off_a + ta; out_b[n] = off_b + tb; }
+}
+
+int exclusive_scan2_i32(hipStream_t st, const int32_t *a, const int32_t *b, int64_t n, int32_t *ab, int64_t *out_ab, int64_t *out_b) {
+    XM_ARG(n >= 0 && a && b && ab && out_ab && out_b);
+    XM_SCOPE(st);
+    const int64_t n_tiles = (n + SCAN_TILE - 1) / SCAN_TILE;
+    if (n_tiles == 0 || n_tiles > SCAN_SELF_MAX) return XMAP_ERR_CAPACITY;
+    long long *tile = nullptr;
+    XM_HIP(xm_malloc_async((void **)&tile, sizeof(long long) * 2 * (size_t)n_tiles, st));
+    k_tile_sums2<<<dim3((unsigned)n_tiles), dim3(SCAN_THREADS), 0, st>>>(a, b, n, tile);
+    XM_LAUNCH_CHECK();
+    k_tile_scan2_self<<<dim3((unsigned)n_tiles), dim3(SCAN_THREADS), 0, st>>>(a, b, n, tile, ab, (long long *)out_ab, (long long *)out_b);
+    XM_LAUNCH_CHECK();
+    XM_HIP(xm_free_async(tile, st));
+    return XMAP_OK;
+}
+
 template <typename TIn>
 static int exclusive_scan(hipStream_t st, const TIn *in, int64_t *out, int64_t n, int64_t *h_total) {
     XM_ARG(n >= 0);
@@ -166,15 +249,22 @@
     int64_t n_tiles = (n + SCAN_TILE - 1) / SCAN_TILE;
     long long *tile = nullptr;
     XM_HIP(xm_malloc_async((void **)&tile, sizeof(long long) * (size_t)(n_tiles + 1), st));
-    if (n_tiles > 0) {
+    if (n_tiles > 0 && n_tiles <= SCAN_SELF_MAX) {
         k_tile_sums<TIn><<<dim3((unsigned)n_tiles), dim3(SCAN_THREADS), 0, st>>>(in, n, tile);
         XM_LAUNCH_CHECK();
-    }
-    k_scan_tile_sums<<<dim3(1), dim3(SCAN_THREADS), 0, st>>>(tile, n_tiles, (long long *)(out + n));
-    XM_LAUNCH_CHECK();
-    if (n_tiles > 0) {
-        k_tile_scan<TIn><<<dim3((unsigned)n_tiles), dim3(SCAN_THREADS), 0, st>>>(in, n, tile, (long long *)out);
+        k_tile_scan_self<TIn><<<dim3((unsigned)n_tiles), dim3(SCAN_THREADS), 0, st>>>(in, n, tile, (long long *)out);
         XM_LAUNCH_CHECK();
+    } else {
+        if (n_tiles > 0) {
+            k_tile_sums<TIn><<<dim3((unsigned)n_tiles), dim3(SCAN_THREADS), 0, st>>>(in, n, tile);
+            XM_LAUNCH_CHECK();
+        }
+        k_scan_tile_sums<<<dim3(1), dim3(SCAN_THREADS), 0, st>>>(tile, n_tiles, (long long *)(out + n));
+        XM_LAUNCH_CHECK();
+        if (n_tiles > 0) {
+            k_tile_scan<TIn><<<dim3((unsigned)n_tiles), dim3(SCAN_THREADS), 0, st>>>(in, n, tile, (long long *)out);
+            XM_LAUNCH_CHECK();
+        }
     }
     XM_HIP(xm_free_async(tile, st));
     if (h_total) {
@@ -183,11 +273,66 @@
     }
     return XMAP_OK;
 }
+
+namespace {
+constexpr int HOST_RING = 8;
+struct HostRing { int dev; char *pin; hipEvent_t ev[HOST_RING]; unsigned gen[HOST_RING]; unsigned next; };
+thread_local std::vector<HostRing *> g_rings;
+HostRing *host_ring() {
+    int dev = 0;
+    if (hipGetDevice(&dev) != hipSuccess) { set_error("hipGetDevice failed"); return nullptr; }
+    for (HostRing *r : g_rings) if (r->dev == dev) return r;
+    HostRing *r = new HostRing();
+    r->dev = dev; r->next = 0;
+    bool ok = hipHostMalloc((void **)&r->pin, (size_t)HOST_RING * XM_HOST_SLOT_BYTES, hipHostMallocDefault) == hipSuccess;
+    for (int s = 0; s < HOST_RING && ok; s++) {
+        r->gen[s] = 0;
+        ok = hipEventCreateWithFlags(&r->ev[s], hipEventDisableTiming) == hipSuccess;
+    }
+    if (!ok) { set_error("could not create the pinned read-back slots"); delete r; return nullptr; }
+    g_rings.push_back(r);
+    return r;
+}
+}
+
+int host_post(hipStream_t st, const void *d_src, size_t bytes, int *ticket) {
+    XM_ARG(d_src && ticket && bytes > 0 && bytes <= XM_HOST_SLOT_BYTES);
+    HostRing *r = host_ring();
+    if (!r) return XMAP_ERR_HIP;
+    const int s = (int)(r->next++ % HOST_RING);
+    r->gen[s] = (r->gen[s] + 1) & 0xffffffu;
+    *ticket = (int)(r->gen[s] << 3) | s;
+    XM_HIP(hipMemcpyAsync(r->pin + (size_t)s * XM_HOST_SLOT_BYTES, d_src, bytes, hipMemcpyDeviceToHost, st));
+    XM_HIP(hipEventRecord(r->ev[s], st));
+    return XMAP_OK;
+}
+int host_wait(int ticket, void *dst, size_t bytes) {
+    XM_ARG(dst && ticket >= 0 && bytes > 0 && bytes <= XM_HOST_SLOT_BYTES);
+    HostRing *r = host_ring();
+    if (!r) return XMAP_ERR_HIP;
+    const int s = ticket & (HOST_RING - 1);
+    if (r->gen[s] == 0 || r->gen[s] != (unsigned)(ticket >> 3)) {
+        set_error("read-back ticket %d is stale (its slot was posted again)", ticket);
+        return XMAP_ERR_ARG;
+    }
+    XM_HIP(hipEventSynchronize(r->ev[s]));
+    memcpy(dst, r->pin + (size_t)s * XM_HOST_SLOT_BYTES, bytes);
+    return XMAP_OK;
+}
 }
 
 extern "C" {
 const char *xmap_last_error(void) { return xmap::g_err; }
-int xmap_version(void) { return 101; }
+int xmap_version(void) { return 102; }
+
+int xmap_host_post(void *stream, const int64_t *d_words, int32_t n_words, int32_t *ticket) {
+    XM_ARG(n_words > 0 && (size_t)n_words * sizeof(int64_t) <= xmap::XM_HOST_SLOT_BYTES);
+    return xmap::host_post((hipStream_t)stream, d_words, sizeof(int64_t) * (size_t)n_words, ticket);
+}
+int xmap_host_wait(int32_t ticket, int64_t *h_words, int32_t n_words) {
+    XM_ARG(n_words > 0 && (size_t)n_words * sizeof(int64_t) <= xmap::XM_HOST_SLOT_BYTES);
+    return xmap::host_wait(ticket, h_words, sizeof(int64_t) * (size_t)n_words);
+}
 
 int xmap_trim(void) {
     XM_HIP(hipDeviceSynchronize());
diff --git a/x-map_amd/xmap/engine/device.py b/x-map_amd/xmap/engine/device.py
--- a/x-map_amd/xmap/engine/device.py
+++ b/x-map_amd/xmap/engine/device.py
@@ -382,6 +382,17 @@
     def _tri_plan3(self, L, slot_target):
         R = self.R
         st = _stream(self.dev)
+        cap_light, cap_heavy = self._plan3_alloc(L, slot_target)
+        h = (C.c_int64 * 10)()
+        with self.timed("tri_plan"):
+            check(lib.xmap_sim3_plan(st, C.byref(R.c), i32(slot_target), vp(L.pre), vp(L.hid), vp(L.ctl), vp(L.Q), vp(L.C),
+                                     vp(L.small), vp(L.Wp), vp(L.Qcat), vp(L.uq_ptr), vp(L.uc_ptr),
+                                     i32(1 if getattr(L, "dups", False) else 0), vp(L.uq_item), vp(L.uq_q), vp(L.uc_item),
+                                     vp(L.uc_c), i64(cap_light), i64(cap_heavy), h))
+        self._plan3_take(L, h, slot_target)
+
+    def _plan3_alloc(self, L, slot_target):
+        R = self.R
         I = R.n_items
         L.Q = self._out(max(I, 1), torch.int32, I > 0)
         L.C = self._out(max(I, 1), torch.int32, I > 0)
@@ -395,12 +406,9 @@
         L.uq_q = self._empty(4 * cap_light, torch.int32)
         L.uc_item = self._empty(cap_heavy, torch.int32)
         L.uc_c = self._empty(cap_heavy, torch.int32)
-        h = (C.c_int64 * 10)()
-        with self.timed("tri_plan"):
-            check(lib.xmap_sim3_plan(st, C.byref(R.c), i32(slot_target), vp(L.pre), vp(L.hid), vp(L.ctl), vp(L.Q), vp(L.C),
-                                     vp(L.small), vp(L.Wp), vp(L.Qcat), vp(L.uq_ptr), vp(L.uc_ptr),
-                                     i32(1 if getattr(L, "dups", False) else 0), vp(L.uq_item), vp(L.uq_q), vp(L.uc_item),
-                                     vp(L.uc_c), i64(cap_light), i64(cap_heavy), h))
+        return cap_light, cap_heavy
+
+    def _plan3_take(self, L, h, slot_target):
         L.n_light, L.n_heavy_units = int(h[0]), int(h[1])
         L.cls_ptr = (C.c_int64 * 6)(*[int(h[2 + c]) for c in range(6)])
         L.CH, L.n_heavy = int(h[8]), int(h[9])
@@ -413,7 +421,7 @@
         return L._heavy_half
 
     def tri_pairs(self, method, cap, stats, L, unit_range=None, do_heavy=True, retry=True, rec=False, raw=False, split=False,
-                  heavy_deal=None, marks=True, count_mir=False):
+                  heavy_deal=None, marks=True, count_mir=False, mirror_pre=None):
         R = self.R
         st = _stream(self.dev)
         m = self.pair_method(method)
@@ -462,11 +470,20 @@
                 with self.timed("pair_tri"):
                     run(8 | 2 | 16 | 64 | (5 if do_heavy else 0) | (32 if raw else 0))
             if count_mir and split and not raw:
+                scratch = self._empty(cap_coo, torch.int32)
+                ticket = C.c_int32(-1)
+                check(lib.xmap_host_post(st, vp(d_cnt), i32(6), C.byref(ticket)))
                 with self.timed("mir_count"):
-                    scratch = self._empty(cap_coo, torch.int32)
                     check(lib.xmap_sim3_mircount(st, i32(I), i64(cap_coo), vp(coo_i), vp(coo_j), vp(d_shards), i64(cap_coo),
                                                  i32(1 if rec else 0), vp(scratch), vp(mircnt)))
-            h = d_cnt.tolist()
+                if mirror_pre is not None:
+                    mirror_pre.update(row_ptr=self._out(I + 1, torch.int64, I > 0), mptr=self._empty(I + 1, torch.int64),
+                                      tot=self._empty(max(I, 1), torch.int32), fill=self._empty(max(I, 1), torch.int32))
+                hw = (C.c_int64 * 6)()
+                check(lib.xmap_host_wait(ticket, hw, i32(6)))
+                h = list(hw)
+            else:
+                h = d_cnt.tolist()
             if h[2]:
                 if L.slot_target <= 32:
                     raise abi.XmapError(abi.ERR_OVERFLOW, "pair-table overflow")
@@ -526,8 +543,10 @@
             coo, rowcnt, n, n_unordered = self.tri_pairs("adjust_cosine", cap, stats, L, do_heavy=False, rec=True)
             S = self.tri_scatter(coo, rowcnt, info, n, L)
         else:
-            coo, own, n, n_unordered, mir, shards = self.tri_pairs("adjust_cosine", cap, stats, L, do_heavy=False, rec=True, split=True, marks=False, count_mir=True)
-            S = self.tri_mirror(coo, own, mir, info, n, shards, counted=True)
+            pre = {}
+            coo, own, n, n_unordered, mir, shards = self.tri_pairs("adjust_cosine", cap, stats, L, do_heavy=False, rec=True, split=True, marks=False,
+                                                                   count_mir=True, mirror_pre=pre)
+            S = self.tri_mirror(coo, own, mir, info, n, shards, counted=True, pre=pre)
         S.cap, S.n_unordered, S.layout = int(cap), n_unordered, L
         S.norm = self.norms[R.n_items:2 * R.n_items]
         return S
@@ -582,9 +601,16 @@
         L.ch_min = int(ch_min)
         L.half_contrib = R.half_contrib
         if item_range is None:
+            cap_light, cap_heavy = self._plan3_alloc(L, slot_target)
+            h = (C.c_int64 * 10)()
             with self.timed("layout3"):
-                call(1 | 2 | 4, 0, I)
-            self._tri_plan3(L, slot_target)
+                check(lib.xmap_sim4_layout_plan(st, C.byref(R.c), vp(R.item_ptr), vp(r64), i32(ch_min), vp(cnt), vp(u_avg), vp(u_norm),
+                                                vp(L.hist), vp(L.pre), vp(L.ctl), vp(L.hid), vp(L.hlist), vp(L.ub_key), vp(L.ub), vp(srec),
+                                                vp(buf_a), vp(buf_b), vp(L.rc), vp(L.Wp), vp(info), vp(self.norms), i32(slot_target),
+                                                vp(L.Q), vp(L.C), vp(L.small), vp(L.Qcat), vp(L.uq_ptr), vp(L.uc_ptr),
+                                                i32(1 if L.dups else 0), vp(L.uq_item), vp(L.uq_q), vp(L.uc_item), vp(L.uc_c),
+                                                i64(cap_light), i64(cap_heavy), h))
+            self._plan3_take(L, h, slot_target)
         else:
             with self.timed("layout3"):
                 call(1 | 2, int(item_range[0]), int(item_range[1]))
@@ -603,7 +629,7 @@
                                      vp(shards), i64(n), i32(1 if skip_self else 0), vp(scratch), vp(mir)))
         return mir
 
-    def tri_mirror(self, coo, own, mir, info, n, shards=None, rows=None, counted=False):
+    def tri_mirror(self, coo, own, mir, info, n, shards=None, rows=None, counted=False, pre=None):
         R = self.R
         st = _stream(self.dev)
         I = R.n_items
@@ -620,10 +646,13 @@
                 mir[:lo].zero_(); mir[hi:].zero_()
                 kept = int((own[lo:hi].long().sum() + mir[lo:hi].long().sum()).item())
         rw = 4 if coo_ls is not None else 3
-        row_ptr = self._out(I + 1, torch.int64, I > 0)
-        mptr = self._empty(I + 1, torch.int64)
-        tot = self._empty(max(I, 1), torch.int32)
-        fill = self._empty(max(I, 1), torch.int32)
+        if pre:
+            row_ptr, mptr, tot, fill = pre["row_ptr"], pre["mptr"], pre["tot"], pre["fill"]
+        else:
+            row_ptr = self._out(I + 1, torch.int64, I > 0)
+            mptr = self._empty(I + 1, torch.int64)
+            tot = self._empty(max(I, 1), torch.int32)
+            fill = self._empty(max(I, 1), torch.int32)
         buf_a = self._empty(max(int(n), 1) * rw, torch.int64)
         buf_b = self._empty(max(int(n), 1) * rw, torch.int64)
         col = self._empty(max(kept, 1), torch.int32)
@@ -656,8 +685,10 @@
             S = self.tri_scatter(coo, rowcnt, stats[2], n, L)
         else:
             stats, L = self.layout3(slot_target, ch_min)
-            coo, rowcnt, n, n_unordered, mir, shards = self.tri_pairs(method, cap, stats, L, split=True, marks=False, count_mir=True)
-            S = self.tri_mirror(coo, rowcnt, mir, stats[2], n, shards, counted=True)
+            pre = {}
+            coo, rowcnt, n, n_unordered, mir, shards = self.tri_pairs(method, cap, stats, L, split=True, marks=False, count_mir=True,
+                                                                      mirror_pre=pre)
+            S = self.tri_mirror(coo, rowcnt, mir, stats[2], n, shards, counted=True, pre=pre)
         S.method = abi.METHODS[method] if isinstance(method, str) else int(method)
         S.cap = int(cap)
         S.u_avg, S.u_norm = stats[0], stats[1]
diff --git a/x-map_amd/xmap/engine/hipabi.py b/x-map_amd/xmap/engine/hipabi.py
--- a/x-map_amd/xmap/engine/hipabi.py
+++ b/x-map_amd/xmap/engine/hipabi.py
@@ -60,6 +60,7 @@
 
 EXPORTS = [
     "xmap_last_error", "xmap_version", "xmap_trim", "xmap_debug_arena", "xmap_debug_arena_call", "xmap_exclusive_scan_i64", "xmap_exclusive_scan_i32_to_i64",
+    "xmap_host_post", "xmap_host_wait", "xmap_sim4_layout_plan",
     "xmap_build_csc", "xmap_user_stats", "xmap_item_stats", 
     "xmap_sim2_layout", "xmap_sim2_plan", "xmap_sim2_units",
     "xmap_sim2_pairs", "xmap_sim2_scatter", "xmap_sim3_layout", "xmap_sim3_plan", "xmap_sim3_mircount", "xmap_sim3_mirror", "xmap_item_partials", "xmap_item_merge", "xmap_sim2_pack_partials",
```
